# HPC-Research-Lab/GNN

Measured on AMD Instinct MI355X. Metric: mini-batches/sec + SpMM HBM GB/s, Reddit GraphSAGE/LADIES at 1/2/4/8 MI355X, higher is better.
Workload: dtype f32

## Files before the change

### gnn_amd/_lib.py

```python
from __future__ import annotations

import contextlib
import ctypes
import os
import threading

import torch

_HERE = os.path.dirname(os.path.abspath(__file__))
LIB_PATH = os.environ.get("GNN_SPMM_LIBRARY") or os.path.join(_HERE, "libgnn_spmm.so")

_lock = threading.Lock()
_lib = None

c_i32p = ctypes.c_void_p
_VP = ctypes.c_void_p
_I64 = ctypes.c_int64
_SZ = ctypes.c_size_t
_INT = ctypes.c_int

_SIGNATURES = {
    "gnn_last_error": (ctypes.c_char_p, []),
    "gnn_version": (ctypes.c_char_p, []),
    "gnn_spmm_default_unit_nnz": (_I64, [_I64, _I64, _I64]),
    "gnn_spmm_workspace_bytes": (_SZ, [_I64, _I64, _I64, _I64]),
    "gnn_spmm_csr_f32": (_INT, [_VP, _VP, _VP, _I64, _I64, _I64, _VP, _I64, _VP, _I64, _I64, _VP, _SZ, _I64, _VP]),
    "gnn_spmm_csr_f32_ex": (_INT, [_VP, _VP, _VP, _I64, _I64, _I64, _VP, _I64, _VP, _I64, _I64, _VP, _I64, _VP,
                                   _VP, _SZ, _I64, _VP]),
    "gnn_spmm_kernel_name": (_INT, [_I64, _I64, _I64, _I64, _I64, _I64, _VP, _VP, _I64, _INT, ctypes.c_char_p, _SZ]),
    "gnn_spmm_config":(_INT, [_I64, _I64, _I64, _I64, _I64, _I64, _VP, _VP, _I64, ctypes.POINTER(ctypes.c_int32)]),
    "gnn_spmm_csr_h16_f32": (_INT, [_VP, _VP, _VP, _I64, _I64, _I64, _VP, _I64, _INT, _VP, _I64, _I64, _VP, _SZ, _I64,
                                    _VP]),
    "gnn_spmm_h16_config": (_INT, [_I64, _I64, _I64, _I64, _I64, _I64, _VP, _VP, _I64,
                                   ctypes.POINTER(ctypes.c_int32)]),
    "gnn_spmm_graph_workspace_bytes": (_SZ, [_I64, _I64, _I64]),
    "gnn_spmm_graph_f32": (_INT, [_VP, _VP, _VP, _I64, _I64, _I64, _I64, _I64, _VP, _I64, _INT, _VP, _I64, _I64, _VP,
                                  _SZ, _VP]),
    "gnn_spmm_rows_workspace_bytes": (_SZ, [_I64, _I64, _I64]),
    "gnn_spmm_rows_f32": (_INT, [_VP, _VP, _VP, _I64, _VP, _I64, _VP, _I64, _VP, _I64, _VP, _I64, _INT, _VP, _I64, _I64,
                                 _VP, _SZ, _VP, _VP]),
    "gnn_closure_table_bytes": (_SZ, [_I64]),
    "gnn_closure_workspace_bytes": (_SZ, [_I64]),
    "gnn_closure_mark": (_INT, [_VP, _VP, _I64, _VP, _I64, ctypes.c_int32, _VP, _VP, _VP, _SZ, _VP]),
    "gnn_closure_list": (_INT, [_VP, _I64, _VP, _I64, _VP]),
    "gnn_closure_rank": (_INT, [_VP, _I64, _VP, _I64, _VP, _VP, _VP]),
    "gnn_nbr_workspace_bytes": (_SZ, [_I64]),
    "gnn_nbr_rowptr": (_INT, [_VP, _I64, _I64, _VP, _I64, ctypes.c_int32, _VP, _VP, _VP, _SZ, _VP, _VP]),
    "gnn_nbr_draw": (_INT, [_VP, _VP, _I64, _I64, _VP, _I64, ctypes.c_int32, ctypes.c_uint64, ctypes.c_int32, _VP, _VP,
                            _VP, _I64, _VP, _VP]),
    "gnn_nbr_relabel": (_INT, [_VP, _I64, _VP, _I64, _VP, _VP, _VP, _VP]),
    "gnn_lw_race": (_INT, [_VP, _VP, _I64, _I64, _VP, _I64, _VP, ctypes.c_uint64, ctypes.c_int32, _VP, _VP, _I64, _VP,
                           _VP, _VP]),
    "gnn_lw_select_workspace_bytes": (_SZ, []),
    "gnn_lw_select": (_INT, [_VP, _VP, _VP, _I64, _I64, _VP, _VP, _VP, _VP, _VP, _SZ, _VP]),
    "gnn_lw_finish_workspace_bytes": (_SZ, [_I64, _I64]),
    "gnn_lw_finish": (_INT, [_VP, _I64, _VP, _I64, _I64, _VP, _I64, _VP, _VP, _I64, _VP, _VP, _I64, _VP, _VP, _VP, _VP,
                             _VP, _VP, _VP, _VP, _SZ, _VP, _VP]),
    "gnn_spmm_set_timing_events": (None, [_VP, _VP]),
    "gnn_segsort_workspace_bytes": (_SZ, [_I64]),
    "gnn_build_operand_workspace_bytes": (_SZ, []),
    "gnn_build_operand_f32": (_INT, [_VP, _VP, _VP, _INT, _VP, _I64, _I64, _I64, _VP, _VP, _VP, _VP, _SZ, _VP]),
    "gnn_build_operand_t_f32": (_INT, [_VP, _VP, _VP, _VP, _I64, _I64, _I64, _VP, _VP]),
    "gnn_build_operand_sorted_f32": (_INT, [_VP, _VP, _VP, _INT, _VP, _I64, _I64, _I64, _VP, _VP, _VP, _VP]),
    "gnn_coo_to_csr": (_INT, [_VP, _VP, _I64, _I64, _VP, _VP, _VP]),
    "gnn_csr_transpose_workspace_bytes": (_SZ, [_I64, _I64, _I64]),
    "gnn_csr_transpose": (_INT, [_VP, _VP, _VP, _I64, _I64, _I64, _VP, _VP, _VP, _VP, _SZ, _VP]),
    "gnn_gather_rows_f32": (_INT, [_VP, _I64, _VP, _VP, _I64, _VP, _I64, _I64, _VP]),
    "gnn_gather_rows2_f32": (_INT, [_VP, _I64, _VP, _VP, _I64, _VP, _I64, _VP, _VP, _I64, _VP, _I64, _I64, _VP]),
    "gnn_gather_rows_h16_f32": (_INT, [_VP, _I64, _INT, _VP, _VP, _I64, _VP, _I64, _I64, _VP]),
    "gnn_gather_rows2_h16_f32": (_INT, [_VP, _I64, _VP, _VP, _I64, _VP, _I64, _VP, _VP, _I64, _INT, _VP, _I64, _I64,
                                        _VP]),
    "gnn_gather_rows_host_f32": (_INT, [_VP, _I64, _VP, _VP, _I64, _VP, _I64, _I64, _VP]),
    "gnn_gather_placed_f32": (_INT, [_VP, _I64, _VP, _INT, _VP, _I64, _INT, _VP, _I64, _VP, _I64, _I64, _VP, _VP, _VP]),
    "gnn_host_register": (_INT, [_VP, _SZ]),
    "gnn_host_unregister": (_INT, [_VP]),
    "gnn_memcpy_h2d_async": (_INT, [_VP, _VP, _SZ, _VP]),
    "gnn_stage_plan": (_SZ, [_VP, _VP]),
    "gnn_stage_batch_f32": (_INT, [_VP, _VP]),
    "gnn_stream_create_cu_masked": (_INT, [ctypes.c_int32, ctypes.c_int32, ctypes.c_int32, ctypes.POINTER(_VP)]),
    "gnn_stream_destroy": (_INT, [_VP]),
    "gnn_ipc_export": (_INT, [_VP, _VP, ctypes.POINTER(_I64)]),
    "gnn_ipc_open": (_INT, [_VP, _I64, _INT, ctypes.POINTER(_VP)]),
    "gnn_ipc_close": (_INT, [_VP, _I64]),
    "gnn_sage_norm_fwd_f32": (_INT, [_VP, _I64, _I64, _VP, _I64, _I64, _VP, _VP, _VP, _VP, _I64, ctypes.c_float,
                                     ctypes.c_uint64, _INT, _VP, _I64, _VP, _VP, _VP]),
    "gnn_sage_norm_bwd_workspace_bytes": (_SZ, [_I64, _I64]),
    "gnn_sage_norm_bwd_f32": (_INT, [_VP, _I64, _VP, _I64, _I64, _VP, _I64, _I64, _VP, _VP, _VP, _VP, _VP, _I64,
                                     ctypes.c_float, ctypes.c_uint64, _INT, _VP, _VP, _VP, _VP, _VP, _VP, _VP, _SZ,
                                     _VP]),
    "gnn_sage_norm_bwd_agg_f32": (_INT, [_VP, _VP, _VP, _VP, _I64, _VP, _I64, _VP, _VP, _I64, _I64, _VP, _I64, _I64,
                                         _VP, _VP, _VP, _VP, _VP, _I64, ctypes.c_float, ctypes.c_uint64, _INT, _VP,
                                         _VP, _VP, _VP, _VP, _VP, _VP, _SZ, _VP]),
    "gnn_sage_norm_config": (_INT, [_I64, _I64, _INT, ctypes.POINTER(ctypes.c_int), ctypes.POINTER(ctypes.c_int),
                                    ctypes.POINTER(ctypes.c_int)]),
    "gnn_gemm_p3_packed_bytes": (_SZ, [_I64, _I64]),
    "gnn_gemm_p3_pack_f32": (_INT, [_VP, _I64, _INT, _VP, _I64, _I64, _VP, _SZ, _VP]),
    "gnn_gemm_p3_workspace_bytes": (_SZ, [_I64, _I64, _I64, _INT]),
    "gnn_gemm_p3": (_INT, [_I64, _I64, _I64, _INT, _VP, _VP, _VP, _I64, _VP, _SZ, _VP]),
    "gnn_optim_chunks": (_I64, [_INT, _VP]),
    "gnn_grad_sqnorm_f32": (_INT, [_INT, _VP, _VP, _VP, _VP]),
    "gnn_clip_scale_f32": (_INT, [_VP, _I64, ctypes.c_float, _VP, _VP]),
    "gnn_scale_into_f32": (_INT, [_INT, _VP, _VP, _VP, _VP, _VP]),
    "gnn_adam_f32": (_INT, [_INT, _VP, _VP, _VP, _VP, _VP, _VP, ctypes.c_float, ctypes.c_float, ctypes.c_float,
                            ctypes.c_float, _I64, _VP]),
    "gnn_head_bce_fwd_f32": (_INT, [_VP, _I64, _I64, _I64, _VP, _VP, _I64, _VP, _I64, ctypes.c_float,
                                    ctypes.c_uint64, _INT, _VP, _VP, _VP, _VP, _VP, _VP]),
    "gnn_head_bce_bwd_f32": (_INT, [_VP, _I64, _I64, _I64, _VP, _I64, _VP, _I64, _VP, ctypes.c_float,
                                    ctypes.c_uint64, _INT, _VP, _VP, _VP, _VP, _I64, _VP]),
    "gnn_head_bias_grad_f32": (_INT, [_VP, _I64, _I64, _VP, _VP]),
    "gnn_head_eval_f32": (_INT, [_VP, _I64, _I64, _I64, _VP, _VP, _I64, _VP, _I64, _VP, _I64, _VP, _VP, _VP, _VP, _INT,
                                 _VP]),
    "gnn_head_ce_fwd_f32": (_INT, [_VP, _I64, _I64, _I64, _VP, _VP, _I64, _VP, _I64, ctypes.c_float,
                                   ctypes.c_uint64, _INT, _VP, _VP, _VP, _VP, _VP, _VP, _VP]),
    "gnn_head_ce_bwd_f32": (_INT, [_VP, _I64, _I64, _I64, _VP, _I64, _VP, _I64, _VP, ctypes.c_float,
                                   ctypes.c_uint64, _INT, _VP, _VP, _VP, _VP, _I64, _VP, _VP]),
    "gnn_head_eval_loss_f32": (_INT, [_VP, _I64, _I64, _I64, _VP, _VP, _I64, _VP, _I64, _VP, _I64, _VP, _VP, _VP, _VP,
                                      _INT, _INT, _VP]),
    "gnn_ladies_extract_workspace_bytes": (_SZ, [_I64, _I64, _I64, ctypes.c_int32, _I64, _I64]),
    "gnn_colcount_create": (_INT, [ctypes.c_int32, _I64, _VP, _VP, ctypes.POINTER(_VP)]),
    "gnn_colcount_add": (_INT, [_VP, _VP, _I64, ctypes.POINTER(_I64), ctypes.POINTER(_VP), ctypes.POINTER(_VP)]),
    "gnn_colcount_reset": (_INT, [_VP]),
    "gnn_colcount_destroy": (None, [_VP]),
    "gnn_colcount_set_cus": (_INT, [ctypes.c_int32]),
    "gnn_ladies_extract_f32": (_INT, [_VP, _VP, _VP, _I64, _VP, _VP, _VP, _I64, _VP, _I64, _VP, _I64, _VP, _VP, _VP, _I64,
                                      _I64, _VP, _VP, _VP, _VP, _VP, _VP, _SZ, _VP, _VP]),
    "gnn_train_step_workspace_bytes": (_SZ, [_VP]),
    "gnn_train_step_f32": (_INT, [_VP, _VP, _SZ, _VP]),
    "gnn_eval_step_workspace_bytes": (_SZ, [_VP]),
    "gnn_eval_step_f32": (_INT, [_VP, _VP, _I64, _VP, _INT, _VP, _SZ, _VP]),
    "gnn_gemm_f32_workspace_bytes": (_SZ, [_I64, _I64, _I64, _INT]),
    "gnn_gemm_f32": (_INT, [_INT, _INT, _I64, _I64, _I64, _INT, _VP, _I64, _VP, _I64, _VP, _I64, _VP, _SZ, _VP]),
    "gnn_gemm_f32_split3_workspace_bytes": (_SZ, [_I64, _I64, _I64, _INT]),
    "gnn_gemm_f32_split3_indexed": (_INT, [_INT, _INT, _I64, _I64, _I64, _INT, _VP, _I64, _VP, _I64, _VP, _I64, _VP,
                                           _I64, _VP, _I64, _VP, _SZ, _VP]),
    "gnn_gemm_f32_split3": (_INT, [_INT, _INT, _I64, _I64, _I64, _INT, _VP, _I64, _VP, _I64, _VP, _I64, _VP, _SZ,
                                   _VP]),
    "gnn_gemm_f32_split_workspace_bytes": (_SZ, [_INT, _I64, _I64, _I64, _INT]),
    "gnn_gemm_f32_split": (_INT, [_INT, _INT, _INT, _I64, _I64, _I64, _INT, _VP, _I64, _VP, _I64, _VP, _I64, _VP, _SZ,
                                  _VP]),
    "gnn_gemm_f32_split_indexed": (_INT, [_INT, _INT, _INT, _I64, _I64, _I64, _INT, _VP, _I64, _VP, _I64, _VP, _I64,
                                          _VP, _I64, _VP, _I64, _VP, _SZ, _VP]),
}

EXPORTED_SYMBOLS = tuple(_SIGNATURES)

SAMPLER_PATH = os.path.join(_HERE, "libgnn_sampler.so")
_SAMPLER_SIGNATURES = {
    "gnn_sampler_last_error": (ctypes.c_char_p, []),
    "gnn_ladies_sample": (_INT, [_VP, _VP, _VP, _I64, _VP, _I64, _VP, _VP, ctypes.c_int32, ctypes.c_uint32,
                                 ctypes.POINTER(_VP)]),
    "gnn_ladies_sample_dev": (_INT, [_VP, _VP, _VP, _VP, _I64, _VP, _I64, _VP, _VP, ctypes.c_int32, ctypes.c_uint32,
                                     ctypes.c_int32, ctypes.POINTER(_VP)]),
    "gnn_ladies_layer_device": (_INT, [_VP, ctypes.c_int32, _VP, _VP, _VP, _VP, _VP]),
    "gnn_subgraph_sample": (_INT, [_VP, _VP, _VP, _I64, _VP, _I64, _VP, _VP, ctypes.c_int32, ctypes.c_uint32,
                                   ctypes.POINTER(_VP)]),
    "gnn_fastgcn_sample": (_INT, [_VP, _VP, _VP, _I64, _VP, _VP, _I64, _VP, _VP, ctypes.c_int32, ctypes.c_uint32,
                                  ctypes.POINTER(_VP)]),
    "gnn_fastgcn_p_changed": (None, []),
    "gnn_ladies_layer_dims": (_INT, [_VP, ctypes.c_int32, ctypes.POINTER(_I64)]),
    "gnn_ladies_layer_copy": (_INT, [_VP, ctypes.c_int32, _VP, _VP, _VP, _VP, _VP]),
    "gnn_ladies_layer_csc": (_INT, [_VP, ctypes.c_int32, _VP, _VP]),
    "gnn_ladies_num_input_nodes": (_I64, [_VP]),
    "gnn_ladies_input_nodes": (_INT, [_VP, _VP]),
    "gnn_ladies_free": (None, [_VP]),
    "gnn_mt19937_random_sample": (_INT, [ctypes.c_uint32, _I64, _VP]),
    "gnn_sampler_profile": (_INT, [_VP, ctypes.c_int32, ctypes.c_int32]),
    "gnn_host_gather_rows_f32": (_INT, [_VP, _I64, _I64, _VP, _I64, _I64, _VP, _I64]),
    "gnn_host_gather_rows_b16": (_INT, [_VP, _I64, _I64, _VP, _I64, _I64, _VP, _I64]),
    "gnn_loader_set_feat_b16": (_INT, [_VP, _VP, _I64, _I64, _I64, ctypes.c_int32]),
    "gnn_loader_create": (_VP, [_VP, _VP, _VP, _VP, _I64, _VP, _VP, _VP, _I64, _VP, _VP, ctypes.c_int32, ctypes.c_int32,
                                _VP, _VP, _I64, _I64, _I64, _VP, _VP, ctypes.c_int32, ctypes.c_int32, _VP,
                                ctypes.c_int32, ctypes.c_int32, ctypes.c_int32, ctypes.c_int32]),
    "gnn_loader_submit": (_INT, [_VP, ctypes.c_uint32, _VP, _I64]),
    "gnn_loader_set_colcount": (_INT, [_VP, _VP]),
    "gnn_loader_set_colcount_workers": (_INT, [_VP, ctypes.c_int32]),
    "gnn_ladies_sample_cc": (_INT, [_VP, _VP, _VP, _VP, _I64, _VP, _I64, _VP, _VP, ctypes.c_int32, ctypes.c_uint32,
                                    ctypes.c_int32, _VP, _VP, ctypes.POINTER(_VP)]),
    "gnn_loader_next": (_INT, [_VP, ctypes.POINTER(_VP)]),
    "gnn_batch_desc": (ctypes.POINTER(_I64), [_VP, ctypes.POINTER(_I64)]),
    "gnn_batch_blob": (_VP, [_VP]),
    "gnn_batch_release": (None, [_VP]),
    "gnn_loader_destroy": (None, [_VP]),
}
SAMPLER_EXPORTED_SYMBOLS = tuple(_SAMPLER_SIGNATURES)
_sampler = None


def lib() -> ctypes.CDLL:
    global _lib
    if _lib is not None:
        return _lib
    with _lock:
        if _lib is None:
            if not os.path.exists(LIB_PATH):
                raise RuntimeError(
                    f"gnn_amd: native library {LIB_PATH} is missing; build it with "
                    "`python -c 'import __graft_entry__ as g; g.build()'` (hipcc, gfx950)")
            handle = ctypes.CDLL(LIB_PATH)
            for name, (res, args) in _SIGNATURES.items():
                fn = getattr(handle, name)
                fn.restype = res
                fn.argtypes = args
            _lib = handle
    return _lib


def sampler_lib() -> ctypes.CDLL:
    global _sampler
    if _sampler is not None:
        return _sampler
    with _lock:
        if _sampler is None:
            if not os.path.exists(SAMPLER_PATH):
                raise RuntimeError(f"gnn_amd: native sampler {SAMPLER_PATH} is missing; build it with "
                                   "`python -c 'import __graft_entry__ as g; g.build()'`")
            handle = ctypes.CDLL(SAMPLER_PATH)
            for name, (res, args) in _SAMPLER_SIGNATURES.items():
                fn = getattr(handle, name)
                fn.restype = res
                fn.argtypes = args
            _sampler = handle
    return _sampler


def check_sampler(rc: int, what: str) -> None:
    if rc != 0:
        msg = sampler_lib().gnn_sampler_last_error().decode(errors="replace")
        raise RuntimeError(f"{what} failed (status {rc}): {msg}")


_NULLCTX = contextlib.nullcontext()


def stream_of(dev) -> int:
    return torch._C._cuda_getCurrentRawStream(dev.index if dev.index is not None else torch.cuda.current_device())


def on_device(dev):
    if dev.index is None or dev.index == torch._C._cuda_getDevice():
        return _NULLCTX
    return torch.cuda.device(dev)


def check(rc: int, what: str) -> None:
    if rc != 0:
        msg = lib().gnn_last_error().decode(errors="replace")
        raise RuntimeError(f"{what} failed (status {rc}): {msg}")
```

### gnn_amd/csrc/common.h

```cpp
#pragma once

#include <hip/hip_runtime.h>

#include <cstddef>
#include <cstdint>

#define GNN_EINVAL (-22)

namespace gnn {

int fail(int code, const char* fmt, ...);

inline size_t align_up(size_t x, size_t a) { return (x + a - 1) / a * a; }
inline int64_t ceil_div(int64_t a, int64_t b) { return (a + b - 1) / b; }

inline int pick_vw(int64_t F, int64_t ldx, int64_t ldy, const void* X, const void* Y) {
  const uintptr_t px = (uintptr_t)X, py = (uintptr_t)Y;
  if (F % 4 == 0 && ldx % 4 == 0 && ldy % 4 == 0 && px % 16 == 0 && py % 16 == 0) return 4;
  if (F % 2 == 0 && ldx % 2 == 0 && ldy % 2 == 0 && px % 8 == 0 && py % 8 == 0) return 2;
  return 1;
}

int launch_scan_exclusive(const int* in, int n, int* out, hipStream_t st);

bool spmm_row_chain(int64_t M, int64_t K, int64_t nnz, int64_t F, int64_t ldx, int64_t ldy, const void* X,
                    const void* Y);

int gemm_split3_as_batch(int a_kmajor, int b_kmajor, int64_t M, int64_t N, int64_t K, int nbatch, int split_nbatch,
                         int batch_index, const float* const* A, int64_t lda, const float* const* B, int64_t ldb,
                         float* const* C, int64_t ldc, void* workspace, size_t workspace_bytes, void* stream,
                         int pieces = 3);

int gemm_split3_indexed(int a_kmajor, int b_kmajor, int64_t M, int64_t N, int64_t K, int nbatch,
                        const float* const* A, int64_t lda, const int64_t* const* ia, int64_t a_rows,
                        const float* const* B, int64_t ldb, const int64_t* const* ib, int64_t b_rows,
                        float* const* C, int64_t ldc, void* workspace, size_t workspace_bytes, void* stream,
                        int pieces = 3);

}

#define GNN_REQUIRE(cond, ...)                              \
  do {                                                      \
    if (!(cond)) return ::gnn::fail(GNN_EINVAL, __VA_ARGS__); \
  } while (0)

#define GNN_LAUNCHED(name)                                                                       \
  do {                                                                                           \
    hipError_t e_ = hipGetLastError();                                                           \
    if (e_ != hipSuccess) return ::gnn::fail((int)e_, "%s launch: %s", name, hipGetErrorString(e_)); \
  } while (0)

#define GNN_HIP(call, name)                                                                \
  do {                                                                                     \
    hipError_t e_ = (call);                                                                \
    if (e_ != hipSuccess) {                                                                \
      (void)hipGetLastError();                                                             \
      return ::gnn::fail((int)e_, "%s: %s", name, hipGetErrorString(e_));                  \
    }                                                                                      \
  } while (0)
```

### gnn_amd/csrc/gemm.hip

```cpp
#include <hip/hip_runtime.h>

#include <algorithm>
#include <climits>
#include <cstdint>
#include <cstdlib>

#include "common.h"
#include "gnn_layers.h"

namespace {

using gnn::ceil_div;

typedef float f2 __attribute__((ext_vector_type(2)));
typedef float f4 __attribute__((ext_vector_type(4)));
typedef float f16v __attribute__((ext_vector_type(16)));

constexpr int BM = 128, BN = 128;
constexpr int KM_LD = BM + 32;
constexpr int MAX_BATCH = 4;

template <int BKT>
struct Stage {
  static constexpr int MM_LD = BKT + 2;
  static constexpr int FLOATS = (BKT * KM_LD > BM * MM_LD) ? BKT * KM_LD : BM * MM_LD;
  static constexpr int NP = BKT / 8;
};

struct Batch {
  const float* A[MAX_BATCH];
  const float* B[MAX_BATCH];
  float* C[MAX_BATCH];
  const int64_t* ia[MAX_BATCH];
  const int64_t* ib[MAX_BATCH];
};

template <int VEC>
__device__ __forceinline__ f4 load4(const float* p) {
  if constexpr (VEC == 4) {
    return *reinterpret_cast<const f4*>(p);
  } else {
    const f2 lo = *reinterpret_cast<const f2*>(p);
    const f2 hi = *reinterpret_cast<const f2*>(p + 2);
    return f4{lo.x, lo.y, hi.x, hi.y};
  }
}

template <bool KMAJ, int VEC, int BKT, bool GUARD>
__device__ __forceinline__ void load_tile(const float* __restrict__ P, int64_t ld, int r0, int rlim, int k0, int klim,
                                          int t, f4 v[Stage<BKT>::NP]) {
#pragma unroll
  for (int j = 0; j < Stage<BKT>::NP; ++j) {
    if constexpr (KMAJ) {
      const int k = k0 + (t >> 5) + 8 * j;
      const int m = r0 + (t & 31) * 4;
      if constexpr (!GUARD) {
        const float* row = P + (int64_t)k * ld;
        if constexpr (VEC == 4) {
          v[j] = load4<4>(row + min(m, ((rlim - 1) >> 2) << 2));
        } else {
          const int mc = ((rlim - 1) >> 1) << 1;
          const f2 lo = *reinterpret_cast<const f2*>(row + min(m, mc));
          const f2 hi = *reinterpret_cast<const f2*>(row + min(m + 2, mc));
          v[j] = f4{lo.x, lo.y, hi.x, hi.y};
        }
      } else {
        f4 x = f4(0.0f);
        if (k < klim) {
          const float* row = P + (int64_t)k * ld;
          if (m + 0 < rlim) x.x = row[m + 0];
          if (m + 1 < rlim) x.y = row[m + 1];
          if (m + 2 < rlim) x.z = row[m + 2];
          if (m + 3 < rlim) x.w = row[m + 3];
        }
        v[j] = x;
      }
    } else {
      constexpr int TPR = BKT / 4;
      const int m = min(r0 + t / TPR + (256 / TPR) * j, rlim - 1);
      const int k = k0 + (t % TPR) * 4;
      const float* q = P + (int64_t)m * ld + k;
      if constexpr (!GUARD) {
        v[j] = load4<VEC>(q);
      } else {
        f4 x = f4(0.0f);
        if (k + 0 < klim) x.x = q[0];
        if (k + 1 < klim) x.y = q[1];
        if (k + 2 < klim) x.z = q[2];
        if (k + 3 < klim) x.w = q[3];
        v[j] = x;
      }
    }
  }
}

template <bool KMAJ, int BKT>
__device__ __forceinline__ void store_tile(float* __restrict__ S, int t, const f4 v[Stage<BKT>::NP]) {
#pragma unroll
  for (int j = 0; j < Stage<BKT>::NP; ++j) {
    if constexpr (KMAJ) {
      const int kk = (t >> 5) + 8 * j, m = (t & 31) * 4;
      *reinterpret_cast<f4*>(S + kk * KM_LD + m) = v[j];
    } else {
      constexpr int TPR = BKT / 4;
      const int m = t / TPR + (256 / TPR) * j, kk = (t % TPR) * 4;
      float* p = S + m * Stage<BKT>::MM_LD + kk;
      *reinterpret_cast<f2*>(p) = f2{v[j].x, v[j].y};
      *reinterpret_cast<f2*>(p + 2) = f2{v[j].z, v[j].w};
    }
  }
}

template <bool KMAJ, int BKT>
__device__ __forceinline__ float frag(const float* __restrict__ S, int r, int k) {
  if constexpr (KMAJ) return S[k * KM_LD + r];
  else return S[r * Stage<BKT>::MM_LD + k];
}

template <int NB>
__device__ __forceinline__ void store_acc(const f16v (&acc)[2][NB], float* Cb, int64_t ldo, int M, int N, int m0,
                                          int n0, int wm, int wn, int li, int lh) {
#pragma unroll
  for (int i = 0; i < 2; ++i) {
#pragma unroll
    for (int j = 0; j < NB; ++j) {
      const int n = n0 + wn * (32 * NB) + j * 32 + li;
      if (n >= N) continue;
#pragma unroll
      for (int r = 0; r < 16; ++r) {
        const int m = (m0 + wm * 64 + i * 32 + (r & 3) + 8 * (r >> 2)) | (4 * lh);
        if (m < M) Cb[(int64_t)m * ldo + n] = acc[i][j][r];
      }
    }
  }
}

template <bool AK, bool BKM, int VA, int VB, int BKT>
__global__ __launch_bounds__(256) void gemm_f32_kernel(Batch bt, int M, int N, int K, int64_t lda, int64_t ldb,
                                                          int64_t ldc, int splits, int klen, float* __restrict__ part) {
  __shared__ __attribute__((aligned(16))) float As[2][Stage<BKT>::FLOATS];
  __shared__ __attribute__((aligned(16))) float Bs[2][Stage<BKT>::FLOATS];
  const int t = threadIdx.x;
  const int lane = t & 63;
  const int wid = t >> 6;
  const int wm = wid >> 1, wn = wid & 1;
  const int b = blockIdx.z / splits;
  const int split = blockIdx.z % splits;
  const int m0 = blockIdx.y * BM;
  const int n0 = blockIdx.x * BN;
  const int kbeg = split * klen;
  const int kend = min(K, kbeg + klen);
  const float* __restrict__ A = bt.A[b];
  const float* __restrict__ B = bt.B[b];

  f16v acc[2][2];
#pragma unroll
  for (int i = 0; i < 2; ++i)
#pragma unroll
    for (int j = 0; j < 2; ++j) acc[i][j] = f16v(0.0f);

  const int nk = kend > kbeg ? (kend - kbeg + BKT - 1) / BKT : 0;
  f4 ra[Stage<BKT>::NP], rb[Stage<BKT>::NP];
  auto load_ab = [&](int k0) {
    if (k0 + BKT <= kend) {
      load_tile<AK, VA, BKT, false>(A, lda, m0, M, k0, kend, t, ra);
      load_tile<BKM, VB, BKT, false>(B, ldb, n0, N, k0, kend, t, rb);
    } else {
      load_tile<AK, VA, BKT, true>(A, lda, m0, M, k0, kend, t, ra);
      load_tile<BKM, VB, BKT, true>(B, ldb, n0, N, k0, kend, t, rb);
    }
  };
  if (nk > 0) {
    load_ab(kbeg);
    store_tile<AK, BKT>(As[0], t, ra);
    store_tile<BKM, BKT>(Bs[0], t, rb);
  }
  __syncthreads();
  const int li = lane & 31, lk = lane >> 5;
  for (int kt = 0; kt < nk; ++kt) {
    const int cur = kt & 1;
    if (kt + 1 < nk) load_ab(kbeg + (kt + 1) * BKT);
    const float* Sa = As[cur];
    const float* Sb = Bs[cur];
#pragma unroll
    for (int s = 0; s < BKT / 2; ++s) {
      const int k = 2 * s + lk;
      const float a0 = frag<AK, BKT>(Sa, wm * 64 + li, k);
      const float a1 = frag<AK, BKT>(Sa, wm * 64 + 32 + li, k);
      const float b0 = frag<BKM, BKT>(Sb, wn * 64 + li, k);
      const float b1 = frag<BKM, BKT>(Sb, wn * 64 + 32 + li, k);
      acc[0][0] = __builtin_amdgcn_mfma_f32_32x32x2f32(a0, b0, acc[0][0], 0, 0, 0);
      acc[0][1] = __builtin_amdgcn_mfma_f32_32x32x2f32(a0, b1, acc[0][1], 0, 0, 0);
      acc[1][0] = __builtin_amdgcn_mfma_f32_32x32x2f32(a1, b0, acc[1][0], 0, 0, 0);
      acc[1][1] = __builtin_amdgcn_mfma_f32_32x32x2f32(a1, b1, acc[1][1], 0, 0, 0);
    }
    if (kt + 1 < nk) {
      store_tile<AK, BKT>(As[cur ^ 1], t, ra);
      store_tile<BKM, BKT>(Bs[cur ^ 1], t, rb);
    }
    __syncthreads();
  }
  store_acc<2>(acc, splits > 1 ? part + (int64_t)blockIdx.z * M * N : bt.C[b], splits > 1 ? N : ldc, M, N, m0, n0, wm,
               wn, li, lk);
}

__global__ __launch_bounds__(256) void gemm_splitk_reduce4_kernel(Batch bt, const float* __restrict__ part, int64_t MN,
                                                                  int splits, int nbatch) {
  const int64_t n4 = MN / 4;
  for (int64_t e = (int64_t)blockIdx.x * 256 + threadIdx.x; e < n4 * nbatch; e += (int64_t)gridDim.x * 256) {
    const int b = (int)(e / n4);
    const int64_t o = (e - (int64_t)b * n4) * 4;
    const float* p = part + (int64_t)b * splits * MN + o;
    f4 acc = *reinterpret_cast<const f4*>(p);
    int q = 1;
    for (; q + 3 < splits; q += 4) {
      const f4 v0 = *reinterpret_cast<const f4*>(p + (int64_t)q * MN);
      const f4 v1 = *reinterpret_cast<const f4*>(p + (int64_t)(q + 1) * MN);
      const f4 v2 = *reinterpret_cast<const f4*>(p + (int64_t)(q + 2) * MN);
      const f4 v3 = *reinterpret_cast<const f4*>(p + (int64_t)(q + 3) * MN);
      acc += v0;
      acc += v1;
      acc += v2;
      acc += v3;
    }
    for (; q < splits; ++q) acc += *reinterpret_cast<const f4*>(p + (int64_t)q * MN);
    *reinterpret_cast<f4*>(bt.C[b] + o) = acc;
  }
}

__global__ __launch_bounds__(256) void gemm_splitk_reduce_kernel(Batch bt, const float* __restrict__ part, int M, int N,
                                                                 int64_t ldc, int splits, int nbatch) {
  const int64_t MN = (int64_t)M * N;
  for (int64_t e = (int64_t)blockIdx.x * 256 + threadIdx.x; e < MN * nbatch; e += (int64_t)gridDim.x * 256) {
    const int b = (int)(e / MN);
    const int64_t o = e - (int64_t)b * MN;
    const float* p = part + (int64_t)b * splits * MN + o;
    float s = p[0];
    for (int q = 1; q < splits; ++q) s += p[(int64_t)q * MN];
    const int m = (int)(o / N), n = (int)(o - (int64_t)m * N);
    bt.C[b][(int64_t)m * ldc + n] = s;
  }
}

typedef __bf16 bf8v __attribute__((ext_vector_type(8)));
typedef unsigned int u4v __attribute__((ext_vector_type(4)));

constexpr int S3_BK = 16;
constexpr int S3_PIECE = BM * S3_BK;
constexpr int S3_OPER = 3 * S3_PIECE;

__device__ __forceinline__ __amdgpu_buffer_rsrc_t s3_rsrc(const float* p, int64_t bytes) {
  return __builtin_amdgcn_make_buffer_rsrc((void*)p, (short)0, (int)bytes, 0x00020000);
}

template <bool KMAJ, int VEC, bool GUARD, bool IX = false>
__device__ __forceinline__ void s3_load(__amdgpu_buffer_rsrc_t rs, const float* __restrict__ P, int64_t ld, int voff,
                                        int r0, int rlim, int k0, int klim, int t, float v[8],
                                        const int64_t* __restrict__ idx = nullptr) {
  if constexpr (KMAJ) {
    const int kb = k0 + __builtin_amdgcn_readfirstlane((t >> 7) * 8);
    if constexpr (GUARD) {
      const int m = min(r0 + (t & 127), rlim - 1);
#pragma unroll
      for (int i = 0; i < 8; ++i)
        v[i] = (kb + i < klim) ? P[(IX ? idx[kb + i] : (int64_t)(kb + i)) * ld + m] : 0.0f;
    } else {
#pragma unroll
      for (int i = 0; i < 8; ++i)
        v[i] = __builtin_bit_cast(
            float, __builtin_amdgcn_raw_buffer_load_b32(
                       rs, voff, (int)((IX ? idx[kb + i] : (int64_t)(kb + i)) * ld * 4), 0));
    }
  } else {
    if constexpr (GUARD) {
      const int m = min(r0 + (t >> 1), rlim - 1);
      const int kb = k0 + (t & 1) * 8;
      const float* q = P + (IX ? idx[m] : (int64_t)m) * ld + kb;
#pragma unroll
      for (int i = 0; i < 8; ++i) v[i] = (kb + i < klim) ? q[i] : 0.0f;
    } else {
      const int so = k0 * 4;
      if constexpr (VEC == 4) {
        const f4 a = __builtin_bit_cast(f4, __builtin_amdgcn_raw_buffer_load_b128(rs, voff, so, 0));
        const f4 b = __builtin_bit_cast(f4, __builtin_amdgcn_raw_buffer_load_b128(rs, voff + 16, so, 0));
        v[0] = a.x; v[1] = a.y; v[2] = a.z; v[3] = a.w;
        v[4] = b.x; v[5] = b.y; v[6] = b.z; v[7] = b.w;
      } else {
#pragma unroll
        for (int i = 0; i < 4; ++i) {
          const f2 a = __builtin_bit_cast(f2, __builtin_amdgcn_raw_buffer_load_b64(rs, voff + 8 * i, so, 0));
          v[2 * i] = a.x;
          v[2 * i + 1] = a.y;
        }
      }
    }
  }
}

template <bool KMAJ>
__device__ __forceinline__ int s3_voff(int64_t ld, int r0, int rlim, int t, const int64_t* __restrict__ idx = nullptr) {
  if constexpr (KMAJ) return min(r0 + (t & 127), rlim - 1) * 4;
  else {
    const int r = min(r0 + (t >> 1), rlim - 1);
    return (int)(((idx ? idx[r] : (int64_t)r) * ld + (t & 1) * 8) * 4);
  }
}

template <bool KMAJ, int R>
__device__ __forceinline__ int s3_chunk(int row, int h) {
  if constexpr (KMAJ) return (h * R + row) * 8;
  else return (2 * row + (h ^ ((row >> 3) & 1))) * 8;
}

typedef __bf16 bf2v __attribute__((ext_vector_type(2)));

__device__ __forceinline__ unsigned int rne_pk(float a, float b) {
  return __builtin_bit_cast(unsigned int, __builtin_convertvector(f2{a, b}, bf2v));
}

template <int NP = 3>
__device__ __forceinline__ void split8(const float v[8], u4v& ph, u4v& pm, u4v& pl) {
  if constexpr (NP == 1) {
#pragma unroll
    for (int j = 0; j < 4; ++j) ph[j] = rne_pk(v[2 * j], v[2 * j + 1]);
    return;
  } else if constexpr (NP == 2) {
#pragma unroll
    for (int j = 0; j < 4; ++j) {
      const float x0 = v[2 * j], x1 = v[2 * j + 1];
      const unsigned int h0 = (__float_as_uint(x0) + 0x80u) & 0xffff0000u;
      const unsigned int h1 = (__float_as_uint(x1) + 0x80u) & 0xffff0000u;
      const float r0 = __builtin_amdgcn_fmed3f(x0 - __uint_as_float(h0), 0.0f, x0);
      const float r1 = __builtin_amdgcn_fmed3f(x1 - __uint_as_float(h1), 0.0f, x1);
      ph[j] = __builtin_amdgcn_perm(h1, h0, 0x07060302u);
      pm[j] = rne_pk(r0, r1);
    }
    return;
  }
#pragma unroll
  for (int j = 0; j < 4; ++j) {
    const float x0 = v[2 * j], x1 = v[2 * j + 1];
    const unsigned int h0 = __float_as_uint(x0) & 0xffff0000u, h1 = __float_as_uint(x1) & 0xffff0000u;
    const float r0 = x0 - __uint_as_float(h0), r1 = x1 - __uint_as_float(h1);
    const unsigned int m0 = __float_as_uint(r0) & 0xffff0000u, m1 = __float_as_uint(r1) & 0xffff0000u;
    const float l0 = r0 - __uint_as_float(m0), l1 = r1 - __uint_as_float(m1);
    ph[j] = __builtin_amdgcn_perm(h1, h0, 0x07060302u);
    pm[j] = __builtin_amdgcn_perm(m1, m0, 0x07060302u);
    pl[j] = __builtin_amdgcn_perm(__float_as_uint(l1), __float_as_uint(l0), 0x07060302u);
  }
}

template <bool KMAJ, int R, int NP = 3>
__device__ __forceinline__ void s3_store(unsigned short* __restrict__ S, int rr, int kh, const float v[8]) {
  u4v ph, pm, pl;
  split8<NP>(v, ph, pm, pl);
  const int off = s3_chunk<KMAJ, R>(rr, kh);
  *reinterpret_cast<u4v*>(S + off) = ph;
  if constexpr (NP >= 2) *reinterpret_cast<u4v*>(S + R * S3_BK + off) = pm;
  if constexpr (NP >= 3) *reinterpret_cast<u4v*>(S + 2 * R * S3_BK + off) = pl;
}

template <bool KMAJ, int R, int NP = 3>
__device__ __forceinline__ void s3_store(unsigned short* __restrict__ S, int t, const float v[8]) {
  s3_store<KMAJ, R, NP>(S, KMAJ ? (t & 127) : (t >> 1), KMAJ ? (t >> 7) : (t & 1), v);
}

template <bool KMAJ, int R>
__device__ __forceinline__ bf8v s3_frag(const unsigned short* __restrict__ S, int piece, int row, int h) {
  return __builtin_bit_cast(bf8v, *reinterpret_cast<const u4v*>(S + piece * R * S3_BK + s3_chunk<KMAJ, R>(row, h)));
}

constexpr int s3_products(int np) { return np == 3 ? 6 : np == 2 ? 4 : 1; }
constexpr int s3_piece_a(int np, int q) {
  constexpr int P3[6] = {2, 1, 0, 1, 0, 0}, P2[4] = {1, 1, 0, 0};
  return np == 3 ? P3[q] : np == 2 ? P2[q] : 0;
}
constexpr int s3_piece_b(int np, int q) {
  constexpr int P3[6] = {0, 1, 2, 0, 1, 0}, P2[4] = {1, 0, 1, 0};
  return np == 3 ? P3[q] : np == 2 ? P2[q] : 0;
}

template <bool AK, bool BKM, int NB, int NP = 3>
__device__ __forceinline__ void s3_mma(const unsigned short* __restrict__ Sa, const unsigned short* __restrict__ Sb,
                                       int ra0, int rb0, int li, int lh, f16v (&acc)[2][NB]) {
  constexpr int G = NB == 2 ? 2 : 1;
  bf8v a[2][NP], bb[G][NP];
#pragma unroll
  for (int p = 0; p < NP; ++p)
#pragma unroll
    for (int i = 0; i < 2; ++i) {
      a[i][p] = s3_frag<AK, BM>(Sa, p, ra0 + i * 32 + li, lh);
      if constexpr (G == 2) bb[i][p] = s3_frag<BKM, 64 * NB>(Sb, p, rb0 + i * 32 + li, lh);
    }
#pragma unroll
  for (int j0 = 0; j0 < NB; j0 += G) {
    if constexpr (G == 1) {
#pragma unroll
      for (int p = 0; p < NP; ++p) bb[0][p] = s3_frag<BKM, 64 * NB>(Sb, p, rb0 + j0 * 32 + li, lh);
    }
#pragma unroll
    for (int q = 0; q < s3_products(NP); ++q)
#pragma unroll
      for (int i = 0; i < 2; ++i)
#pragma unroll
        for (int g = 0; g < G; ++g)
          acc[i][j0 + g] = __builtin_amdgcn_mfma_f32_32x32x16_bf16(a[i][s3_piece_a(NP, q)], bb[g][s3_piece_b(NP, q)],
                                                                  acc[i][j0 + g], 0, 0, 0);
  }
}

__device__ __forceinline__ int3 xcd_tile(int gx, int gy, unsigned gz, unsigned bx, unsigned by, unsigned bz) {
  const int total = gx * gy * gz;
  const int hw = bx + gx * (by + gy * bz);
  const int per = total >> 3;
  const int lg = hw < per * 8 ? (hw & 7) * per + (hw >> 3) : hw;
  return make_int3(lg % gx, (lg / gx) % gy, lg / (gx * gy));
}

template <bool AK, bool BKM, int VA, int VB, bool IDX, int NB, int NP = 3>
__global__ __launch_bounds__(256)
    __attribute__((amdgpu_waves_per_eu(NB == 2 ? 3 : 2, NB == 2 ? (NP == 3 ? 3 : 4) : 2))) void
gemm_s3_kernel(Batch bt, int M, int N, int K, int64_t lda, int64_t ldb, int64_t ldc, int splits, int klen,
               float* __restrict__ part, int64_t abytes, int64_t bbytes, int xcd_map, int tail_base = 0,
               int tail_s = 0) {
  constexpr int TN = 64 * NB;
  constexpr int NH = NB / 2;
  static_assert(NP >= 1 && NP <= 3 && (NP == 3 || NB == 2), "reduced piece counts: the 128 x 128 tile only");
  __shared__ __attribute__((aligned(16))) unsigned short As[2][NP * S3_PIECE];
  __shared__ __attribute__((aligned(16))) unsigned short Bs[2][NH * NP * S3_PIECE];
  const int t = threadIdx.x;
  const int lane = t & 63;
  const int wid = t >> 6;
  const int wm = wid >> 1, wn = wid & 1;
  int tx = blockIdx.x, ty = blockIdx.y, tz = blockIdx.z;
  int b, split;
  int piece = -1;
  if (NB == 2 && tail_s > 0) {
    const int gx = (N + BN - 1) / BN, gy = (M + BM - 1) / BM;
    const int hw = blockIdx.x;
    int lg;
    if (hw < tail_base) {
      const int per = tail_base >> 3;
      lg = xcd_map ? (hw & 7) * per + (hw >> 3) : hw;
      split = 0;
    } else {
      piece = hw - tail_base;
      lg = tail_base + piece / tail_s;
      split = piece % tail_s;
    }
    tx = lg % gx;
    ty = (lg / gx) % gy;
    b = lg / (gx * gy);
  } else {
    if (xcd_map) {
      const int3 tile = xcd_tile(gridDim.x, gridDim.y, gridDim.z, blockIdx.x, blockIdx.y, blockIdx.z);
      tx = tile.x, ty = tile.y, tz = tile.z;
    }
    b = tz / splits;
    split = tz % splits;
  }
  const int m0 = ty * BM;
  const int n0 = tx * TN;
  const bool whole = NB == 2 && tail_s > 0 && piece < 0;
  const int kbeg = whole ? 0 : split * klen;
  const int kend = whole ? K : min(K, kbeg + klen);
  const float* __restrict__ A = bt.A[b];
  const float* __restrict__ B = bt.B[b];
  const __amdgpu_buffer_rsrc_t rsa = s3_rsrc(A, abytes), rsb = s3_rsrc(B, bbytes);
  const int64_t* __restrict__ ia = (IDX && !AK) ? bt.ia[b] : nullptr;
  const int64_t* __restrict__ ib = (IDX && BKM) ? bt.ib[b] : nullptr;
  const int voa = s3_voff<AK>(lda, m0, M, t, ia);
  const int vob0 = s3_voff<BKM>(ldb, n0, N, t);
  const int vob1 = NH == 2 ? s3_voff<BKM>(ldb, n0 + BN, N, t) : 0;

  const int ar = AK ? (t & 127) : (t >> 1), ah = AK ? (t >> 7) : (t & 1);
  const int br = BKM ? (t & 127) : (t >> 1), bh = BKM ? (t >> 7) : (t & 1);
  f16v acc[2][NB];
#pragma unroll
  for (int i = 0; i < 2; ++i)
#pragma unroll
    for (int j = 0; j < NB; ++j) acc[i][j] = f16v(0.0f);

  float ra[2][8], rb[2][8 * NH];
  const int nfull = (kend - kbeg) / S3_BK;
  auto load_ab = [&](int kt, float(&xa)[8], float(&xb)[8 * NH]) {
    const int k0 = kbeg + min(kt, nfull - 1) * S3_BK;
    s3_load<AK, VA, false>(rsa, A, lda, voa, m0, M, k0, kend, t, xa);
    if (IDX && BKM && ib)
      s3_load<BKM, VB, false, true>(rsb, B, ldb, vob0, n0, N, k0, kend, t, xb, ib);
    else
      s3_load<BKM, VB, false>(rsb, B, ldb, vob0, n0, N, k0, kend, t, xb);
    if constexpr (NH == 2) {
      if (IDX && BKM && ib)
        s3_load<BKM, VB, false, true>(rsb, B, ldb, vob1, n0 + BN, N, k0, kend, t, xb + 8, ib);
      else
        s3_load<BKM, VB, false>(rsb, B, ldb, vob1, n0 + BN, N, k0, kend, t, xb + 8);
    }
  };
  auto store_ab = [&](int stage, const float(&xa)[8], const float(&xb)[8 * NH]) {
    if constexpr (NH == 2) {
      s3_store<AK, BM, NP>(As[stage], ar, ah, xa);
      s3_store<BKM, TN, NP>(Bs[stage], br, bh, xb);
      s3_store<BKM, TN, NP>(Bs[stage], br + BN, bh, xb + 8);
    } else {
      s3_store<AK, BM, NP>(As[stage], t, xa);
      s3_store<BKM, TN, NP>(Bs[stage], t, xb);
    }
  };
  const int li = lane & 31, lh = lane >> 5;
  if (nfull > 0) {
    load_ab(0, ra[0], rb[0]);
    load_ab(1, ra[1], rb[1]);
    store_ab(0, ra[0], rb[0]);
    __syncthreads();
    int kt = 0;
    for (; kt + 1 < nfull; kt += 2) {
      load_ab(kt + 2, ra[0], rb[0]);
      s3_mma<AK, BKM, NB, NP>(As[0], Bs[0], wm * 64, wn * (32 * NB), li, lh, acc);
      store_ab(1, ra[1], rb[1]);
      __syncthreads();
      load_ab(kt + 3, ra[1], rb[1]);
      s3_mma<AK, BKM, NB, NP>(As[1], Bs[1], wm * 64, wn * (32 * NB), li, lh, acc);
      store_ab(0, ra[0], rb[0]);
      __syncthreads();
    }
    if (nfull & 1) {
      s3_mma<AK, BKM, NB, NP>(As[0], Bs[0], wm * 64, wn * (32 * NB), li, lh, acc);
      __syncthreads();
    }
  }
  if (kbeg + nfull * S3_BK < kend) {
    const int k0 = kbeg + nfull * S3_BK;
    if (IDX && !AK && ia)
      s3_load<AK, VA, true, true>(rsa, A, lda, voa, m0, M, k0, kend, t, ra[0], ia);
    else
      s3_load<AK, VA, true>(rsa, A, lda, voa, m0, M, k0, kend, t, ra[0]);
    if (IDX && BKM && ib)
      s3_load<BKM, VB, true, true>(rsb, B, ldb, vob0, n0, N, k0, kend, t, rb[0], ib);
    else
      s3_load<BKM, VB, true>(rsb, B, ldb, vob0, n0, N, k0, kend, t, rb[0]);
    if constexpr (NH == 2) {
      if (IDX && BKM && ib)
        s3_load<BKM, VB, true, true>(rsb, B, ldb, vob1, n0 + BN, N, k0, kend, t, rb[0] + 8, ib);
      else
        s3_load<BKM, VB, true>(rsb, B, ldb, vob1, n0 + BN, N, k0, kend, t, rb[0] + 8);
    }
    store_ab(0, ra[0], rb[0]);
    __syncthreads();
    s3_mma<AK, BKM, NB, NP>(As[0], Bs[0], wm * 64, wn * (32 * NB), li, lh, acc);
  }

  if constexpr (NB == 2) {
    if (piece >= 0) {
      float* __restrict__ P = part + (int64_t)piece * (BM * BN);
#pragma unroll
      for (int i = 0; i < 2; ++i)
#pragma unroll
        for (int j = 0; j < 2; ++j)
#pragma unroll
          for (int r = 0; r < 16; ++r)
            P[(wm * 64 + i * 32 + (r & 3) + 8 * (r >> 2) + 4 * lh) * BN + wn * 64 + j * 32 + li] = acc[i][j][r];
      return;
    }
  }
  store_acc<NB>(acc, splits > 1 ? part + (int64_t)tz * M * N : bt.C[b], splits > 1 ? N : ldc, M, N, m0, n0, wm, wn, li,
                lh);
}


__global__ __launch_bounds__(256) void gemm_tail_reduce_kernel(Batch bt, const float* __restrict__ part, int M, int N,
                                                               int64_t ldc, int tail_base, int tail_s) {
  const int tile = blockIdx.x >> 4;
  const int e4 = (blockIdx.x & 15) * 256 + threadIdx.x;
  const int ml = e4 >> 5, nl = (e4 & 31) * 4;
  const float* p = part + (int64_t)tile * tail_s * (BM * BN) + ml * BN + nl;
  f4 acc = *reinterpret_cast<const f4*>(p);
  for (int q = 1; q < tail_s; ++q) acc += *reinterpret_cast<const f4*>(p + (int64_t)q * (BM * BN));
  const int gx = (N + BN - 1) / BN, gy = (M + BM - 1) / BM;
  const int lg = tail_base + tile;
  const int m = ((lg / gx) % gy) * BM + ml, n = (lg % gx) * BN + nl;
  if (m >= M) return;
  float* c = bt.C[lg / (gx * gy)] + (int64_t)m * ldc + n;
  if (n + 0 < N) c[0] = acc.x;
  if (n + 1 < N) c[1] = acc.y;
  if (n + 2 < N) c[2] = acc.z;
  if (n + 3 < N) c[3] = acc.w;
}

__global__ __launch_bounds__(256) void p3_pack_kernel(const float* __restrict__ src, int64_t ld, int kmajor,
                                                      const int64_t* __restrict__ idx, int R, int K, int Rp, int KT,
                                                      unsigned short* __restrict__ out) {
  const int t = threadIdx.x;
  const int r0 = blockIdx.x * 128;
  const int kt = blockIdx.y;
  const int rr = kmajor ? (t & 127) : (t >> 1);
  const int kh = kmajor ? (t >> 7) : (t & 1);
  const int r = r0 + rr;
  const int kb = kt * 16 + kh * 8;
  float v[8];
  if (!kmajor) {
    const float* q = (r < R) ? src + (idx ? idx[r] : (int64_t)r) * ld : nullptr;
#pragma unroll
    for (int i = 0; i < 8; ++i) v[i] = (q && kb + i < K) ? q[kb + i] : 0.0f;
  } else {
#pragma unroll
    for (int i = 0; i < 8; ++i) {
      const int k = kb + i;
      v[i] = (r < R && k < K) ? src[(idx ? idx[k] : (int64_t)k) * ld + r] : 0.0f;
    }
  }
  u4v ph, pm, pl;
  split8(v, ph, pm, pl);
  const int64_t plane = (int64_t)KT * Rp * 16;
  const int64_t o = ((int64_t)kt * Rp + r) * 16 + kh * 8;
  *reinterpret_cast<u4v*>(out + o) = ph;
  *reinterpret_cast<u4v*>(out + plane + o) = pm;
  *reinterpret_cast<u4v*>(out + 2 * plane + o) = pl;
}

struct PBatch {
  const unsigned short* A[MAX_BATCH];
  const unsigned short* B[MAX_BATCH];
  float* C[MAX_BATCH];
};

__global__ __launch_bounds__(256) __attribute__((amdgpu_waves_per_eu(3, 3))) void gemm_p3_kernel(
    PBatch bt, int M, int N, int Mp, int Np, int KT, int64_t ldc, int splits, int ktlen, float* __restrict__ part,
    int xcd_map) {
  __shared__ __attribute__((aligned(16))) unsigned short As[2][S3_OPER];
  __shared__ __attribute__((aligned(16))) unsigned short Bs[2][S3_OPER];
  const int t = threadIdx.x;
  const int lane = t & 63;
  const int wid = t >> 6;
  const int wm = wid >> 1, wn = wid & 1;
  int tx = blockIdx.x, ty = blockIdx.y, tz = blockIdx.z;
  if (xcd_map) {
    const int3 tile = xcd_tile(gridDim.x, gridDim.y, gridDim.z, blockIdx.x, blockIdx.y, blockIdx.z);
    tx = tile.x, ty = tile.y, tz = tile.z;
  }
  const int b = tz / splits;
  const int split = tz % splits;
  const int m0 = ty * BM;
  const int n0 = tx * BN;
  const int ktb = split * ktlen;
  const int kte = min(KT, ktb + ktlen);
  const int64_t aplane = (int64_t)KT * Mp * 16, bplane = (int64_t)KT * Np * 16;
  const __amdgpu_buffer_rsrc_t rsa = __builtin_amdgcn_make_buffer_rsrc((void*)bt.A[b], (short)0,
                                                                      (int)(3 * aplane * 2), 0x00020000);
  const __amdgpu_buffer_rsrc_t rsb = __builtin_amdgcn_make_buffer_rsrc((void*)bt.B[b], (short)0,
                                                                      (int)(3 * bplane * 2), 0x00020000);
  const int rr = t >> 1, kh = t & 1;
  const int voa = ((m0 + rr) * 16 + kh * 8) * 2, vob = ((n0 + rr) * 16 + kh * 8) * 2;
  const int off = s3_chunk<false, BM>(rr, kh);

  f16v acc[2][2];
#pragma unroll
  for (int i = 0; i < 2; ++i)
#pragma unroll
    for (int j = 0; j < 2; ++j) acc[i][j] = f16v(0.0f);

  u4v ra[2][3], rb[2][3];
  const int nfull = kte - ktb;
  auto load_ab = [&](int kt, u4v(&xa)[3], u4v(&xb)[3]) {
    const int k = ktb + min(kt, nfull - 1);
#pragma unroll
    for (int p = 0; p < 3; ++p) {
      xa[p] = __builtin_bit_cast(u4v, __builtin_amdgcn_raw_buffer_load_b128(
                                          rsa, voa, (int)((p * aplane + (int64_t)k * Mp * 16) * 2), 0));
      xb[p] = __builtin_bit_cast(u4v, __builtin_amdgcn_raw_buffer_load_b128(
                                          rsb, vob, (int)((p * bplane + (int64_t)k * Np * 16) * 2), 0));
    }
  };
  auto store_ab = [&](int stage, const u4v(&xa)[3], const u4v(&xb)[3]) {
#pragma unroll
    for (int p = 0; p < 3; ++p) {
      *reinterpret_cast<u4v*>(As[stage] + p * S3_PIECE + off) = xa[p];
      *reinterpret_cast<u4v*>(Bs[stage] + p * S3_PIECE + off) = xb[p];
    }
  };
  const int li = lane & 31, lh = lane >> 5;
  if (nfull > 0) {
    load_ab(0, ra[0], rb[0]);
    load_ab(1, ra[1], rb[1]);
    store_ab(0, ra[0], rb[0]);
    __syncthreads();
    int kt = 0;
    for (; kt + 1 < nfull; kt += 2) {
      load_ab(kt + 2, ra[0], rb[0]);
      s3_mma<false, false, 2>(As[0], Bs[0], wm * 64, wn * 64, li, lh, acc);
      store_ab(1, ra[1], rb[1]);
      __syncthreads();
      load_ab(kt + 3, ra[1], rb[1]);
      s3_mma<false, false, 2>(As[1], Bs[1], wm * 64, wn * 64, li, lh, acc);
      store_ab(0, ra[0], rb[0]);
      __syncthreads();
    }
    if (nfull & 1) {
      s3_mma<false, false, 2>(As[0], Bs[0], wm * 64, wn * 64, li, lh, acc);
      __syncthreads();
    }
  }
  store_acc<2>(acc, splits > 1 ? part + (int64_t)tz * M * N : bt.C[b], splits > 1 ? N : ldc, M, N, m0, n0, wm, wn, li, lh);
}

constexpr int64_t SLOTS_F32 = 2 * 256;
constexpr int64_t SLOTS_S3 = 3 * 256;

int pick_splits(int64_t M, int64_t N, int64_t K, int nbatch, int64_t tile_n, int64_t slots) {
  if (const char* e = getenv("GNN_GEMM_SPLITS")) return std::max(1, atoi(e));
  const int64_t tiles = ceil_div(M, (int64_t)BM) * ceil_div(N, tile_n) * nbatch;
  if (tiles * 2 > slots) return 1;
  int64_t s = slots / tiles;
  s = std::min<int64_t>(s, std::max<int64_t>(1, K / 256));
  return (int)std::max<int64_t>(1, std::min<int64_t>(s, 64));
}

constexpr int W_BN = 2 * BN;
constexpr int64_t SLOTS_S3W = 2 * 256;

bool use_wide(int64_t M, int64_t N, int64_t K, int nbatch) {
  const char* e = getenv("GNN_GEMM_WIDE");
  const int mode = e ? atoi(e) : 0;
  if (mode == 0 || N < W_BN || K <= 0) return false;
  if (mode == 1) return true;
  if (getenv("GNN_GEMM_SPLITS")) return false;
  const int64_t tw = ceil_div(M, (int64_t)BM) * ceil_div(N, (int64_t)W_BN) * nbatch;
  return tw * 100 >= SLOTS_S3W * 85 && tw <= SLOTS_S3W;
}

struct TailPlan {
  int base = 0;
  int s = 0;
  int rem = 0;
};

TailPlan tail_plan(int64_t M, int64_t N, int64_t K, int nbatch) {
  TailPlan tp;
  const int64_t T = ceil_div(M, (int64_t)BM) * ceil_div(N, (int64_t)BN) * nbatch;
  if (T <= 256 || T >= INT_MAX / 2) return tp;
  const int64_t rem = T % 256;
  if (rem == 0 || rem > 32) return tp;
  const int64_t S = std::min<int64_t>(std::min<int64_t>(256 / rem, 4), ceil_div(K, (int64_t)16) / 4);
  if (S < 2) return tp;
  tp.base = (int)(T - rem);
  tp.s = (int)S;
  tp.rem = (int)rem;
  return tp;
}

bool tail_enabled() {
  const char* e = getenv("GNN_GEMM_TAIL");
  return !(e && atoi(e) == 0);
}

size_t tail_bytes(const TailPlan& tp) { return (size_t)tp.rem * tp.s * BM * BN * sizeof(float); }

enum Algo { ALGO_F32 = 0, ALGO_S3 = 1 };
enum Kern { KERN_F32, KERN_S3, KERN_S3W };

bool xcd_map_enabled() {
  const char* e = getenv("GNN_GEMM_XCD");
  return !e || atoi(e) != 0;
}

struct Plan {
  Kern kern = KERN_F32;
  int splits = 1;
  TailPlan tp;
  size_t bytes(int64_t M, int64_t N, int nbatch) const {
    return splits > 1 ? (size_t)splits * nbatch * M * N * sizeof(float) : tail_bytes(tp);
  }
};

Plan plan_of(int algo, int64_t M, int64_t N, int64_t K, int nbatch, int split_nbatch = 0, int batch_index = -1,
             int pieces = 3) {
  const int nb = split_nbatch > 0 ? split_nbatch : nbatch;
  Plan p;
  p.kern = algo != ALGO_S3 ? KERN_F32 : (pieces == 3 && use_wide(M, N, K, nb)) ? KERN_S3W : KERN_S3;
  if (K > 0)
    p.splits = p.kern == KERN_S3W   ? pick_splits(M, N, K, nb, W_BN, SLOTS_S3W)
               : p.kern == KERN_S3 ? pick_splits(M, N, K, nb, BN, SLOTS_S3)
                                   : pick_splits(M, N, K, nb, BN, SLOTS_F32);
  if (p.kern != KERN_S3 || p.splits > 1 || K <= 0) return p;
  if (split_nbatch == 0) {
    p.tp = tail_plan(M, N, K, nbatch);
  } else if (nbatch == 1 && batch_index >= 0) {
    const TailPlan full = tail_plan(M, N, K, split_nbatch);
    const int64_t T1 = ceil_div(M, (int64_t)BM) * ceil_div(N, (int64_t)BN);
    const int64_t lo = (int64_t)batch_index * T1;
    if (full.s > 0 && full.base < lo + T1) {
      p.tp.base = (int)std::max<int64_t>(0, full.base - lo);
      p.tp.s = full.s;
      p.tp.rem = (int)(T1 - p.tp.base);
    }
  }
  return p;
}

size_t workspace_bytes_of(int algo, int64_t M, int64_t N, int64_t K, int nbatch, int pieces = 3) {
  if (M <= 0 || N <= 0 || K <= 0 || nbatch <= 0) return 0;
  return plan_of(algo, M, N, K, nbatch, 0, -1, pieces).bytes(M, N, nbatch);
}

int launch_splitk_reduce(const Batch& bt, const float* part, int64_t M, int64_t N, int64_t ldc, int splits, int nbatch,
                         hipStream_t st) {
  const int64_t total = M * N * nbatch;
  bool vec4 = ldc == N && (M * N) % 4 == 0;
  for (int b = 0; b < nbatch; ++b) vec4 = vec4 && (uintptr_t)bt.C[b] % 16 == 0;
  if (vec4) {
    const unsigned g = (unsigned)std::min<int64_t>(ceil_div(total / 4, (int64_t)256), 2048);
    gemm_splitk_reduce4_kernel<<<dim3(g), dim3(256), 0, st>>>(bt, part, M * N, splits, nbatch);
    GNN_LAUNCHED("gemm_splitk_reduce4_kernel");
  } else {
    const unsigned g = (unsigned)std::min<int64_t>(ceil_div(total, (int64_t)256), 2048);
    gemm_splitk_reduce_kernel<<<dim3(g), dim3(256), 0, st>>>(bt, part, (int)M, (int)N, ldc, splits, nbatch);
    GNN_LAUNCHED("gemm_splitk_reduce_kernel");
  }
  return 0;
}

struct Launch {
  Kern kern;
  bool idx;
  int np;
  int bkt;
  dim3 grid;
  hipStream_t st;
  Batch bt;
  int M, N, K;
  int64_t lda, ldb, ldc;
  int splits, klen;
  float* part;
  int64_t abytes, bbytes;
  int xcdm, tail_base, tail_s;
};

template <bool AK, bool BKM, int VA, int VB, int NP>
void launch_s3_reduced(const Launch& l) {
  auto k = gemm_s3_kernel<AK, BKM, VA, VB, false, 2, NP>;
  if constexpr (!AK || BKM)
    if (l.idx) k = gemm_s3_kernel<AK, BKM, VA, VB, true, 2, NP>;
  k<<<l.grid, dim3(256), 0, l.st>>>(l.bt, l.M, l.N, l.K, l.lda, l.ldb, l.ldc, l.splits, l.klen, l.part, l.abytes,
                                    l.bbytes, l.xcdm, l.tail_base, l.tail_s);
}

template <bool AK, bool BKM, int VA, int VB>
void launch_gemm(const Launch& l) {
  if (l.kern == KERN_F32) {
    auto k = l.bkt == 16 ? gemm_f32_kernel<AK, BKM, VA, VB, 16> : gemm_f32_kernel<AK, BKM, VA, VB, 32>;
    k<<<l.grid, dim3(256), 0, l.st>>>(l.bt, l.M, l.N, l.K, l.lda, l.ldb, l.ldc, l.splits, l.klen, l.part);
    return;
  }
  if (l.np < 3) {
    constexpr int CVA = AK ? 4 : VA, CVB = BKM ? 4 : VB;
    if (l.np == 2) launch_s3_reduced<AK, BKM, CVA, CVB, 2>(l);
    else launch_s3_reduced<AK, BKM, CVA, CVB, 1>(l);
    return;
  }
  const bool wide = l.kern == KERN_S3W;
  auto k = wide ? gemm_s3_kernel<AK, BKM, VA, VB, false, 4> : gemm_s3_kernel<AK, BKM, VA, VB, false, 2>;
  if constexpr (!AK || BKM)
    if (l.idx) k = wide ? gemm_s3_kernel<AK, BKM, VA, VB, true, 4> : gemm_s3_kernel<AK, BKM, VA, VB, true, 2>;
  k<<<l.grid, dim3(256), 0, l.st>>>(l.bt, l.M, l.N, l.K, l.lda, l.ldb, l.ldc, l.splits, l.klen, l.part, l.abytes,
                                    l.bbytes, l.xcdm, l.tail_base, l.tail_s);
}

template <bool AK, bool BKM>
void launch_gemm(int va, int vb, const Launch& l) {
  if (va == 4 && vb == 4) launch_gemm<AK, BKM, 4, 4>(l);
  else if (va == 4) launch_gemm<AK, BKM, 4, 2>(l);
  else if (vb == 4) launch_gemm<AK, BKM, 2, 4>(l);
  else launch_gemm<AK, BKM, 2, 2>(l);
}

struct RowIndex {
  const int64_t* const* ia = nullptr;
  int64_t a_rows = 0;
  const int64_t* const* ib = nullptr;
  int64_t b_rows = 0;
};

int gemm_run(int algo, int a_kmajor, int b_kmajor, int64_t M, int64_t N, int64_t K, int nbatch, const float* const* A,
             int64_t lda, const float* const* B, int64_t ldb, float* const* C, int64_t ldc, void* workspace,
             size_t workspace_bytes, void* stream, int split_nbatch = 0, const RowIndex* ri = nullptr,
             int batch_index = -1, int pieces = 3) {
  GNN_REQUIRE(pieces >= 1 && pieces <= 3 && (pieces == 3 || algo == ALGO_S3),
              "gnn_gemm_f32_split: pieces %d (1: bf16, 2: split2, 3: split3)", pieces);
  GNN_REQUIRE(M >= 0 && N >= 0 && K >= 0, "gnn_gemm_f32: negative size");
  GNN_REQUIRE(M < INT_MAX && N < INT_MAX && K < INT_MAX, "gnn_gemm_f32: sizes must be < 2^31");
  GNN_REQUIRE(nbatch >= 1 && nbatch <= MAX_BATCH, "gnn_gemm_f32: nbatch must be 1..%d", MAX_BATCH);
  if (M == 0 || N == 0) return 0;
  GNN_REQUIRE(A && B && C, "gnn_gemm_f32: NULL pointer array");
  GNN_REQUIRE(ldc >= N, "gnn_gemm_f32: ldc < N");
  GNN_REQUIRE(lda >= (a_kmajor ? M : K) && ldb >= (b_kmajor ? N : K), "gnn_gemm_f32: lda/ldb too small");
  GNN_REQUIRE(lda % 2 == 0 && ldb % 2 == 0, "gnn_gemm_f32: lda and ldb must be even (8-byte rows)");
  Launch l{};
  Batch& bt = l.bt;
  int va = 4, vb = 4;
  for (int b = 0; b < nbatch; ++b) {
    GNN_REQUIRE(C[b] && (K == 0 || (A[b] && B[b])), "gnn_gemm_f32: NULL operand %d", b);
    GNN_REQUIRE((uintptr_t)A[b] % 8 == 0 && (uintptr_t)B[b] % 8 == 0, "gnn_gemm_f32: A/B not 8-byte aligned");
    if (lda % 4 || (uintptr_t)A[b] % 16) va = 2;
    if (ldb % 4 || (uintptr_t)B[b] % 16) vb = 2;
    bt.A[b] = A[b];
    bt.B[b] = B[b];
    bt.C[b] = C[b];
    bt.ia[b] = ri && ri->ia ? ri->ia[b] : nullptr;
    bt.ib[b] = ri && ri->ib ? ri->ib[b] : nullptr;
  }
  for (int b = 0; b < nbatch; ++b) l.idx = l.idx || bt.ia[b] || bt.ib[b];
  GNN_REQUIRE(!l.idx || (algo == ALGO_S3 && (!ri->ia || !a_kmajor) && (!ri->ib || b_kmajor)),
              "gnn_gemm: row indices need split3, an m-major A or a k-major B");
  const int64_t arows = (ri && ri->ia) ? ri->a_rows : (a_kmajor ? K : M);
  const int64_t brows = (ri && ri->ib) ? ri->b_rows : (b_kmajor ? K : N);
  l.abytes = K == 0 ? 0 : (arows - 1) * lda * 4 + (a_kmajor ? M : K) * 4;
  l.bbytes = K == 0 ? 0 : (brows - 1) * ldb * 4 + (b_kmajor ? N : K) * 4;
  if (algo == ALGO_S3 && (l.abytes >= INT_MAX || l.bbytes >= INT_MAX)) {
    GNN_REQUIRE(!l.idx, "gnn_gemm: indexed operand of >= 2 GiB");
    GNN_REQUIRE(pieces == 3, "gnn_gemm_f32_split: operand of >= 2 GiB at %d pieces", pieces);
    algo = ALGO_F32;
  }
  l.np = pieces;
  Plan pl = plan_of(algo, M, N, K, nbatch, split_nbatch, batch_index, pieces);
  if (!tail_enabled()) pl.tp = TailPlan{};
  const TailPlan& tp = pl.tp;
  l.kern = pl.kern;
  l.splits = pl.splits;
  l.xcdm = xcd_map_enabled() && !(tp.s > 0 && tp.base % 8);
  l.bkt = algo == ALGO_S3 ? S3_BK : 32;
  if (algo == ALGO_F32)
    if (const char* e = getenv("GNN_GEMM_BKT")) l.bkt = atoi(e) == 16 ? 16 : 32;
  const int64_t kpart = tp.s > 0 ? tp.s : l.splits;
  l.klen = kpart > 1 ? (int)(ceil_div(ceil_div(K, kpart), (int64_t)l.bkt) * l.bkt) : (int)K;
  if (l.splits > 1 || tp.s > 0) {
    const size_t need = pl.bytes(M, N, nbatch);
    GNN_REQUIRE(workspace && workspace_bytes >= need, "gnn_gemm_f32: workspace too small (%zu < %zu)",
                workspace_bytes, need);
  }
  l.grid = tp.s > 0 ? dim3((unsigned)(tp.base + tp.rem * tp.s))
                    : dim3((unsigned)ceil_div(N, (int64_t)(l.kern == KERN_S3W ? W_BN : BN)),
                           (unsigned)ceil_div(M, (int64_t)BM), (unsigned)(nbatch * l.splits));
  l.st = (hipStream_t)stream;
  l.M = (int)M, l.N = (int)N, l.K = (int)K;
  l.lda = lda, l.ldb = ldb, l.ldc = ldc;
  l.part = (float*)workspace;
  l.tail_base = tp.base, l.tail_s = tp.s;
  if (a_kmajor && b_kmajor) launch_gemm<true, true>(va, vb, l);
  else if (a_kmajor) launch_gemm<true, false>(va, vb, l);
  else if (b_kmajor) launch_gemm<false, true>(va, vb, l);
  else launch_gemm<false, false>(va, vb, l);
  GNN_LAUNCHED(algo == ALGO_S3 ? "gemm_s3_kernel" : "gemm_f32_kernel");
  if (tp.s > 0) {
    gemm_tail_reduce_kernel<<<dim3((unsigned)(tp.rem * 16)), dim3(256), 0, l.st>>>(bt, l.part, (int)M, (int)N, ldc,
                                                                                  tp.base, tp.s);
    GNN_LAUNCHED("gemm_tail_reduce_kernel");
  }
  if (l.splits > 1) return launch_splitk_reduce(bt, l.part, M, N, ldc, l.splits, nbatch, l.st);
  return 0;
}

}

extern "C" {

size_t gnn_gemm_f32_workspace_bytes(int64_t M, int64_t N, int64_t K, int nbatch) {
  return workspace_bytes_of(ALGO_F32, M, N, K, nbatch);
}

int gnn_gemm_f32(int a_kmajor, int b_kmajor, int64_t M, int64_t N, int64_t K, int nbatch, const float* const* A,
                 int64_t lda, const float* const* B, int64_t ldb, float* const* C, int64_t ldc, void* workspace,
                 size_t workspace_bytes, void* stream) {
  return gemm_run(ALGO_F32, a_kmajor, b_kmajor, M, N, K, nbatch, A, lda, B, ldb, C, ldc, workspace, workspace_bytes,
                  stream);
}

size_t gnn_gemm_p3_packed_bytes(int64_t R, int64_t K) {
  if (R <= 0 || K <= 0) return 0;
  return (size_t)3 * (size_t)ceil_div(K, (int64_t)16) * (size_t)(ceil_div(R, (int64_t)128) * 128) * 16 * 2;
}

int gnn_gemm_p3_pack_f32(const float* src, int64_t ld, int kmajor, const int64_t* idx, int64_t R, int64_t K,
                         void* out, size_t out_bytes, void* stream) {
  GNN_REQUIRE(R >= 0 && K >= 0 && R < INT_MAX && K < INT_MAX, "gnn_gemm_p3_pack_f32: bad size");
  if (R == 0 || K == 0) return 0;
  GNN_REQUIRE(src && out, "gnn_gemm_p3_pack_f32: NULL pointer");
  GNN_REQUIRE(out_bytes >= gnn_gemm_p3_packed_bytes(R, K), "gnn_gemm_p3_pack_f32: output too small");
  GNN_REQUIRE((uintptr_t)out % 16 == 0, "gnn_gemm_p3_pack_f32: output not 16-byte aligned");
  GNN_REQUIRE(gnn_gemm_p3_packed_bytes(R, K) < (size_t)INT_MAX, "gnn_gemm_p3_pack_f32: packed operand >= 2 GiB");
  const int Rp = (int)(ceil_div(R, (int64_t)128) * 128), KT = (int)ceil_div(K, (int64_t)16);
  p3_pack_kernel<<<dim3((unsigned)(Rp / 128), (unsigned)KT), dim3(256), 0, (hipStream_t)stream>>>(
      src, ld, kmajor, idx, (int)R, (int)K, Rp, KT, (unsigned short*)out);
  GNN_LAUNCHED("p3_pack_kernel");
  return 0;
}

size_t gnn_gemm_p3_workspace_bytes(int64_t M, int64_t N, int64_t K, int nbatch) {
  return workspace_bytes_of(ALGO_S3, M, N, K, nbatch);
}

int gnn_gemm_p3(int64_t M, int64_t N, int64_t K, int nbatch, const void* const* Ap, const void* const* Bp,
                float* const* C, int64_t ldc, void* workspace, size_t workspace_bytes, void* stream) {
  GNN_REQUIRE(M >= 0 && N >= 0 && K >= 0 && M < INT_MAX && N < INT_MAX && K < INT_MAX, "gnn_gemm_p3: bad size");
  GNN_REQUIRE(nbatch >= 1 && nbatch <= MAX_BATCH, "gnn_gemm_p3: nbatch must be 1..%d", MAX_BATCH);
  if (M == 0 || N == 0) return 0;
  GNN_REQUIRE(Ap && Bp && C && ldc >= N, "gnn_gemm_p3: NULL pointer array or ldc < N");
  PBatch bt{};
  for (int b = 0; b < nbatch; ++b) {
    GNN_REQUIRE(C[b] && (K == 0 || (Ap[b] && Bp[b])), "gnn_gemm_p3: NULL operand %d", b);
    GNN_REQUIRE((uintptr_t)Ap[b] % 16 == 0 && (uintptr_t)Bp[b] % 16 == 0, "gnn_gemm_p3: packed operands 16-byte aligned");
    bt.A[b] = (const unsigned short*)Ap[b];
    bt.B[b] = (const unsigned short*)Bp[b];
    bt.C[b] = C[b];
  }
  GNN_REQUIRE(gnn_gemm_p3_packed_bytes(M, K) < (size_t)INT_MAX && gnn_gemm_p3_packed_bytes(N, K) < (size_t)INT_MAX,
              "gnn_gemm_p3: packed operand >= 2 GiB");
  hipStream_t st = (hipStream_t)stream;
  const int Mp = (int)(ceil_div(M, (int64_t)128) * 128), Np = (int)(ceil_div(N, (int64_t)128) * 128);
  const int KT = (int)ceil_div(K, (int64_t)16);
  const int splits = K == 0 ? 1 : pick_splits(M, N, K, nbatch, BN, SLOTS_S3);
  const int ktlen = splits > 1 ? (int)ceil_div(ceil_div(K, (int64_t)splits), (int64_t)S3_BK) : KT;
  if (splits > 1) {
    const size_t need = (size_t)splits * nbatch * M * N * sizeof(float);
    GNN_REQUIRE(workspace && workspace_bytes >= need, "gnn_gemm_p3: workspace too small (%zu < %zu)", workspace_bytes,
                need);
  }
  const dim3 grid((unsigned)(Np / BN), (unsigned)(Mp / BM), (unsigned)(nbatch * splits));
  float* part = (float*)workspace;
  gemm_p3_kernel<<<grid, dim3(256), 0, st>>>(bt, (int)M, (int)N, Mp, Np, KT, ldc, splits, ktlen, part,
                                             (int)xcd_map_enabled());
  GNN_LAUNCHED("gemm_p3_kernel");
  if (splits > 1) {
    Batch cb{};
    for (int b = 0; b < nbatch; ++b) cb.C[b] = C[b];
    return launch_splitk_reduce(cb, part, M, N, ldc, splits, nbatch, st);
  }
  return 0;
}

size_t gnn_gemm_f32_split3_workspace_bytes(int64_t M, int64_t N, int64_t K, int nbatch) {
  return workspace_bytes_of(ALGO_S3, M, N, K, nbatch);
}

int gnn_gemm_f32_split3(int a_kmajor, int b_kmajor, int64_t M, int64_t N, int64_t K, int nbatch,
                        const float* const* A, int64_t lda, const float* const* B, int64_t ldb, float* const* C,
                        int64_t ldc, void* workspace, size_t workspace_bytes, void* stream) {
  return gemm_run(ALGO_S3, a_kmajor, b_kmajor, M, N, K, nbatch, A, lda, B, ldb, C, ldc, workspace, workspace_bytes,
                  stream);
}

int gnn_gemm_f32_split3_indexed(int a_kmajor, int b_kmajor, int64_t M, int64_t N, int64_t K, int nbatch,
                                const float* const* A, int64_t lda, const int64_t* const* ia, int64_t a_rows,
                                const float* const* B, int64_t ldb, const int64_t* const* ib, int64_t b_rows,
                                float* const* C, int64_t ldc, void* workspace, size_t workspace_bytes, void* stream) {
  GNN_REQUIRE((!ia || a_rows > 0) && (!ib || b_rows > 0), "gnn_gemm_f32_split3_indexed: source rows");
  return gnn::gemm_split3_indexed(a_kmajor, b_kmajor, M, N, K, nbatch, A, lda, ia, a_rows, B, ldb, ib, b_rows, C, ldc,
                                  workspace, workspace_bytes, stream);
}

size_t gnn_gemm_f32_split_workspace_bytes(int pieces, int64_t M, int64_t N, int64_t K, int nbatch) {
  if (pieces < 1 || pieces > 3) return 0;
  return workspace_bytes_of(ALGO_S3, M, N, K, nbatch, pieces);
}

int gnn_gemm_f32_split(int pieces, int a_kmajor, int b_kmajor, int64_t M, int64_t N, int64_t K, int nbatch,
                       const float* const* A, int64_t lda, const float* const* B, int64_t ldb, float* const* C,
                       int64_t ldc, void* workspace, size_t workspace_bytes, void* stream) {
  return gemm_run(ALGO_S3, a_kmajor, b_kmajor, M, N, K, nbatch, A, lda, B, ldb, C, ldc, workspace, workspace_bytes,
                  stream, 0, nullptr, -1, pieces);
}

int gnn_gemm_f32_split_indexed(int pieces, int a_kmajor, int b_kmajor, int64_t M, int64_t N, int64_t K, int nbatch,
                               const float* const* A, int64_t lda, const int64_t* const* ia, int64_t a_rows,
                               const float* const* B, int64_t ldb, const int64_t* const* ib, int64_t b_rows,
                               float* const* C, int64_t ldc, void* workspace, size_t workspace_bytes, void* stream) {
  GNN_REQUIRE(pieces >= 1 && pieces <= 3, "gnn_gemm_f32_split_indexed: pieces %d (1: bf16, 2: split2, 3: split3)",
              pieces);
  GNN_REQUIRE((!ia || a_rows > 0) && (!ib || b_rows > 0), "gnn_gemm_f32_split_indexed: source rows");
  return gnn::gemm_split3_indexed(a_kmajor, b_kmajor, M, N, K, nbatch, A, lda, ia, a_rows, B, ldb, ib, b_rows, C, ldc,
                                  workspace, workspace_bytes, stream, pieces);
}

}

namespace gnn {

int gemm_split3_as_batch(int a_kmajor, int b_kmajor, int64_t M, int64_t N, int64_t K, int nbatch, int split_nbatch,
                         int batch_index, const float* const* A, int64_t lda, const float* const* B, int64_t ldb,
                         float* const* C, int64_t ldc, void* workspace, size_t workspace_bytes, void* stream,
                         int pieces) {
  return gemm_run(ALGO_S3, a_kmajor, b_kmajor, M, N, K, nbatch, A, lda, B, ldb, C, ldc, workspace, workspace_bytes,
                  stream, split_nbatch, nullptr, batch_index, pieces);
}

int gemm_split3_indexed(int a_kmajor, int b_kmajor, int64_t M, int64_t N, int64_t K, int nbatch,
                        const float* const* A, int64_t lda, const int64_t* const* ia, int64_t a_rows,
                        const float* const* B, int64_t ldb, const int64_t* const* ib, int64_t b_rows,
                        float* const* C, int64_t ldc, void* workspace, size_t workspace_bytes, void* stream,
                        int pieces) {
  RowIndex ri;
  ri.ia = ia;
  ri.a_rows = a_rows;
  ri.ib = ib;
  ri.b_rows = b_rows;
  return gemm_run(ALGO_S3, a_kmajor, b_kmajor, M, N, K, nbatch, A, lda, B, ldb, C, ldc, workspace, workspace_bytes,
                  stream, 0, &ri, -1, pieces);
}

}
```

### gnn_amd/csrc/step.hip

```cpp
#include <hip/hip_runtime.h>
#include <rocblas/rocblas.h>

#include <algorithm>
#include <climits>
#include <cstdint>
#include <cstdlib>
#include <cstring>
#include <memory>
#include <mutex>
#include <string>

#include "common.h"
#include "gnn_layers.h"
#include "gnn_spmm.h"
#include "gnn_step.h"

namespace {

using gnn::align_up;
using gnn::ceil_div;

__global__ __launch_bounds__(256) void colsum_kernel(const float* __restrict__ dz, int M, int C,
                                                     float* __restrict__ out) {
  __shared__ float red[4];
  const int c = blockIdx.x;
  float s = 0.0f;
  for (int r = threadIdx.x; r < M; r += 256) s += dz[(int64_t)r * C + c];
#pragma unroll
  for (int m = 32; m >= 1; m >>= 1) s += __shfl_xor(s, m);
  if ((threadIdx.x & 63) == 0) red[threadIdx.x >> 6] = s;
  __syncthreads();
  if (threadIdx.x == 0) out[c] = (red[0] + red[1]) + (red[2] + red[3]);
}

struct Arena {
  char* base;
  size_t off = 0;
  template <typename T>
  T* take(int64_t count) {
    const size_t bytes = align_up((size_t)(count > 0 ? count : 1) * sizeof(T), 256);
    T* p = base ? (T*)(base + off) : nullptr;
    off += bytes;
    return p;
  }
};

int64_t L(const int64_t* d, int l, int f) { return d[GNN_STEP_HEADER + l * GNN_STEP_LAYER_SLOTS + f]; }
template <typename T>
T* P(const int64_t* d, int l, int f) {
  return (T*)(uintptr_t)L(d, l, f);
}
template <typename T>
T* HP(const int64_t* d, int f) {
  return (T*)(uintptr_t)d[f];
}

bool fills(int64_t M, int64_t N, int n) { return ceil_div(M, 128) * ceil_div(N, 128) * n >= 256; }
bool gemm_ok(const void* p, int64_t ld) { return ((uintptr_t)p % 8) == 0 && (ld % 2) == 0; }

std::mutex g_blas_mu;
rocblas_handle g_blas[64][2] = {};

int blas_handle(rocblas_handle* h, int which = 0) {
  int dev = 0;
  GNN_HIP(hipGetDevice(&dev), "hipGetDevice");
  GNN_REQUIRE(dev >= 0 && dev < 64, "gnn_train_step: device index %d", dev);
  std::lock_guard<std::mutex> g(g_blas_mu);
  if (!g_blas[dev][which]) {
    if (rocblas_create_handle(&g_blas[dev][which]) != rocblas_status_success)
      return gnn::fail(-1, "rocblas_create_handle failed");
  }
  *h = g_blas[dev][which];
  return 0;
}

struct Aux {
  hipStream_t s = nullptr;
  hipEvent_t ev[24] = {};
  int next = 0;
  std::mutex mu;
  hipEvent_t take() { return ev[next++ % 24]; }
};
std::mutex g_aux_mu;
Aux* g_aux[64][4] = {};

int aux_of(hipStream_t st, Aux** out) {
  int dev = 0;
  GNN_HIP(hipGetDevice(&dev), "hipGetDevice");
  GNN_REQUIRE(dev >= 0 && dev < 64, "gnn_train_step: device index %d", dev);
  int prio = 0, lo = 0, hi = 0;
  GNN_HIP(hipStreamGetPriority(st, &prio), "hipStreamGetPriority");
  GNN_HIP(hipDeviceGetStreamPriorityRange(&lo, &hi), "hipDeviceGetStreamPriorityRange");
  const int slot = std::min(3, std::max(0, lo - prio));
  std::lock_guard<std::mutex> g(g_aux_mu);
  Aux*& a = g_aux[dev][slot];
  if (!a) {
    std::unique_ptr<Aux> n(new Aux());
    GNN_HIP(hipStreamCreateWithPriority(&n->s, hipStreamNonBlocking, prio), "hipStreamCreateWithPriority");
    for (auto& e : n->ev) GNN_HIP(hipEventCreateWithFlags(&e, hipEventDisableTiming), "hipEventCreateWithFlags");
    a = n.release();
  }
  *out = a;
  return 0;
}

int fork_join(Aux* a, hipStream_t from, hipStream_t to) {
  hipEvent_t e = a->take();
  GNN_HIP(hipEventRecord(e, from), "hipEventRecord");
  GNN_HIP(hipStreamWaitEvent(to, e, 0), "hipStreamWaitEvent");
  return 0;
}

bool no_index() {
  const char* e = getenv("GNN_STEP_GATHER");
  const char* a = getenv("GNN_GEMM_ALGO");
  return (e && atoi(e) != 0) || (a && std::string(a) == "f32");
}

bool f32_gemm() {
  const char* e = getenv("GNN_GEMM_ALGO");
  return e && std::string(e) == "f32";
}

int pieces_of(int np) {
  if (np) return np;
  const char* e = getenv("GNN_GEMM_ALGO");
  if (!e) return 3;
  const std::string a(e);
  return a == "split2" ? 2 : a == "bf16" ? 1 : 3;
}

int gemm(int np, int ak, int bk, int64_t M, int64_t N, int64_t K, int nb, const float* const* A, int64_t lda,
         const float* const* B, int64_t ldb, float* const* C, int64_t ldc, void* ws, size_t wsb, hipStream_t st) {
  if (np == 0 && f32_gemm()) return gnn_gemm_f32(ak, bk, M, N, K, nb, A, lda, B, ldb, C, ldc, ws, wsb, st);
  return gnn_gemm_f32_split(pieces_of(np), ak, bk, M, N, K, nb, A, lda, B, ldb, C, ldc, ws, wsb, st);
}

size_t gemm_ws(int64_t M, int64_t N, int64_t K, int nb) {
  return std::max({gnn_gemm_f32_split3_workspace_bytes(M, N, K, nb), gnn_gemm_f32_workspace_bytes(M, N, K, nb),
                   gnn_gemm_f32_split_workspace_bytes(2, M, N, K, nb)});
}

bool fuse_agg_enabled() {
  const char* e = getenv("GNN_STEP_FUSE_AGG");
  return !(e && atoi(e) == 0);
}

bool small_overlap_enabled() {
  const char* e = getenv("GNN_STEP_SMALL_OVERLAP");
  return !(e && atoi(e) == 0);
}

bool overlap_enabled() {
  const char* e = getenv("GNN_STEP_OVERLAP");
  return e && atoi(e) != 0;
}

int sgemm(rocblas_handle h, rocblas_operation ta, rocblas_operation tb, int64_t m, int64_t n, int64_t k,
          const float* A, int64_t lda, const float* B, int64_t ldb, float* C, int64_t ldc) {
  const float one = 1.0f, zero = 0.0f;
  if (rocblas_sgemm(h, ta, tb, (rocblas_int)m, (rocblas_int)n, (rocblas_int)k, &one, A, (rocblas_int)lda, B,
                    (rocblas_int)ldb, &zero, C, (rocblas_int)ldc) != rocblas_status_success)
    return gnn::fail(-1, "rocblas_sgemm failed (m %lld n %lld k %lld)", (long long)m, (long long)n, (long long)k);
  return 0;
}
int mm_xwt(rocblas_handle h, const float* x, int64_t ldx, const float* W, int64_t ldw, float* out, int64_t ldo,
           int64_t M, int64_t N, int64_t K) {
  return sgemm(h, rocblas_operation_transpose, rocblas_operation_none, N, M, K, W, ldw, x, ldx, out, ldo);
}
int mm_gw(rocblas_handle h, const float* g, int64_t ldg, const float* W, int64_t ldw, float* out, int64_t ldo,
          int64_t M, int64_t K, int64_t N) {
  return sgemm(h, rocblas_operation_none, rocblas_operation_none, K, M, N, W, ldw, g, ldg, out, ldo);
}
int mm_gtx(rocblas_handle h, const float* g, int64_t ldg, const float* x, int64_t ldx, float* out, int64_t ldo,
           int64_t N, int64_t K, int64_t M) {
  return sgemm(h, rocblas_operation_none, rocblas_operation_transpose, K, N, M, x, ldx, g, ldg, out, ldo);
}

struct LayerBufs {
  int64_t M, K, nnz, F, Fk, ldx, ldo, N, D;
  bool xs_gathered;
  bool dense;
  int np;
  const float* X;
  int xk;
  const void* X16;
  float *feat, *xs, *hB, *hW, *Y, *mean, *rstd;
  float *dY, *dhB, *dhW, *dxs, *dfeat;
  void *ws_fwd, *ws_bwd, *ws_norm, *ws_gemm_f, *ws_gemm_f2, *ws_gemm_dx, *ws_gemm_dw;
  size_t b_fwd, b_bwd, b_norm, b_gemm_f, b_gemm_dx, b_gemm_dw;
  bool dy_agg;
  const int32_t *agg_rp, *agg_col, *agg_rmap;
  const float *agg_val, *agg_G, *agg_R;
  const float* in() const { return xk ? feat : X; }
  int64_t ldin() const { return xk ? ldo : ldx; }
};

struct Plan {
  int nl = 0, sage = 1;
  LayerBufs lb[GNN_STEP_MAX_LAYERS];
  float *xd, *z, *nrm, *rowloss, *lse, *dz, *dXh;
  int loss_kind = GNN_LOSS_BCE;
  uint64_t* rowmask;
  int64_t Mh = 0, Dh = 0, C = 0;
};

#define GNN_TRY(x)        \
  do {                    \
    int rc_ = (x);        \
    if (rc_) return rc_;  \
  } while (0)

int shapes(const int64_t* d, bool measuring, Plan& pl) {
  GNN_REQUIRE(d[GNN_SH_VERSION] == GNN_STEP_VERSION, "gnn_train_step: descriptor version %lld",
              (long long)d[GNN_SH_VERSION]);
  GNN_REQUIRE(d[GNN_SH_LOSS_KIND] == GNN_LOSS_BCE || d[GNN_SH_LOSS_KIND] == GNN_LOSS_CE,
              "gnn_train_step: loss kind %lld (0: BCE, 1: CE)", (long long)d[GNN_SH_LOSS_KIND]);
  pl.loss_kind = (int)d[GNN_SH_LOSS_KIND];
  pl.nl = (int)d[GNN_SH_LAYERS];
  pl.sage = d[GNN_SH_KIND] == GNN_STEP_SAGE;
  GNN_REQUIRE(pl.nl >= 1 && pl.nl <= GNN_STEP_MAX_LAYERS, "gnn_train_step: %d layers", pl.nl);
  const int64_t N = d[GNN_SH_NHID];
  const int n = pl.sage ? 2 : 1;
  for (int l = 0; l < pl.nl; ++l) {
    LayerBufs& b = pl.lb[l];
    b.dy_agg = false;
    b.M = L(d, l, GNN_SL_M);
    b.K = L(d, l, GNN_SL_K);
    b.nnz = L(d, l, GNN_SL_NNZ);
    b.N = N;
    const int64_t dense = L(d, l, GNN_SL_DENSE);
    GNN_REQUIRE(dense == 0 || dense == 1, "gnn_train_step: layer %d dense flag %lld (0: aggregating, 1: order 0)", l,
                (long long)dense);
    b.dense = dense != 0;
    const int64_t np = L(d, l, GNN_SL_GEMM);
    GNN_REQUIRE(np >= 0 && np <= 3,
                "gnn_train_step: layer %d GEMM pieces %lld (0: GNN_GEMM_ALGO, 1: bf16, 2: split2, 3: split3)", l,
                (long long)np);
    b.np = (int)np;
    b.D = b.dense ? N : n * N;
    if (b.dense) {
      GNN_REQUIRE(b.K == b.M, "gnn_train_step: order-0 layer %d has K = %lld, M = %lld", l, (long long)b.K,
                  (long long)b.M);
      b.nnz = 0;
    }
    const int64_t xk = L(d, l, GNN_SL_XKIND);
    GNN_REQUIRE(xk == GNN_FEAT_F32 || (l == 0 && (xk == GNN_FEAT_F16 || xk == GNN_FEAT_BF16)),
                "gnn_train_step: layer %d input kind %lld (0: fp32; 1 fp16 / 2 bf16 on layer 0 only)", l,
                (long long)xk);
    b.xk = (int)xk;
    b.X16 = nullptr;
    if (l == 0) {
      b.X = xk ? nullptr : HP<const float>(d, GNN_SH_X0);
      b.X16 = xk ? HP<const void>(d, GNN_SH_X0) : nullptr;
      b.ldx = d[GNN_SH_LDX0];
      b.F = d[GNN_SH_F0];
    } else {
      const LayerBufs& p = pl.lb[l - 1];
      GNN_REQUIRE(b.K == p.M, "gnn_train_step: layer %d has K = %lld, layer %d M = %lld", l, (long long)b.K, l - 1,
                  (long long)p.M);
      b.X = nullptr;
      b.ldx = p.D;
      b.F = p.D;
    }
    GNN_REQUIRE(b.F <= b.ldx && b.F > 0 && b.M > 0 && b.K > 0, "gnn_train_step: layer %d shape", l);
    b.Fk = b.F;
    if (b.F % 4 && b.ldx % 4 == 0 && (l >= 1 || (uintptr_t)b.X % 16 == 0 || measuring) &&
        b.ldx >= b.F + (4 - b.F % 4))
      b.Fk = b.F + (4 - b.F % 4);
    b.ldo = (b.Fk != b.F && b.ldx <= 2 * b.Fk) ? b.ldx : b.Fk;
    if (xk) {
      GNN_REQUIRE(b.ldx % 4 == 0 && ((uintptr_t)b.X16 % 8 == 0 || measuring),
                  "gnn_train_step: 16-bit x0 needs 8-byte aligned rows (ldx %lld)", (long long)b.ldx);
      b.Fk = (int64_t)align_up((size_t)b.F, 4);
      GNN_REQUIRE(b.Fk <= b.ldx, "gnn_train_step: 16-bit x0 rows of %lld elements have no room for %lld columns",
                  (long long)b.ldx, (long long)b.Fk);
      b.ldo = (int64_t)align_up((size_t)b.Fk, 32);
    }
    b.b_fwd = b.dense ? 0 : gnn_spmm_workspace_bytes(b.M, b.nnz, b.Fk, 0);
    b.b_gemm_f = gemm_ws(b.M, N, b.F, b.dense ? 1 : n);
  }
  const LayerBufs& top = pl.lb[pl.nl - 1];
  pl.Mh = top.M;
  pl.Dh = top.D;
  pl.C = d[GNN_SH_CLASSES];
  GNN_REQUIRE(pl.C > 0 && pl.C <= 256 && pl.Dh % 4 == 0 && pl.Dh <= 2048, "gnn_train_step: head %lld x %lld",
              (long long)pl.Dh, (long long)pl.C);
  return 0;
}

int plan_eval(const int64_t* d, Arena& ar, Plan& pl) {
  GNN_TRY(shapes(d, !ar.base, pl));
  int64_t feat = 0, xs = 0, h = 0, rows = 0, y[2] = {0, 0};
  size_t wf = 0, wg = 0;
  bool agg = false;
  for (int l = 0; l < pl.nl; ++l) {
    const LayerBufs& b = pl.lb[l];
    agg = agg || !b.dense;
    if (!b.dense || b.xk) feat = std::max(feat, b.M * b.ldo);
    if (!b.dense) xs = std::max(xs, b.M * b.ldo);
    h = std::max(h, b.M * b.N);
    rows = std::max(rows, b.M);
    y[l & 1] = std::max(y[l & 1], b.M * b.D);
    wf = std::max(wf, b.b_fwd);
    wg = std::max(wg, b.b_gemm_f);
  }
  LayerBufs s = {};
  const bool pair = pl.sage && agg;
  s.feat = (agg || feat) ? ar.take<float>(feat) : nullptr;
  s.xs = pair ? ar.take<float>(xs) : nullptr;
  s.hB = pair ? ar.take<float>(h) : nullptr;
  s.hW = ar.take<float>(h);
  float* const Y[2] = {ar.take<float>(y[0]), ar.take<float>(y[1])};
  s.mean = ar.take<float>(rows);
  s.rstd = ar.take<float>(rows);
  s.ws_fwd = agg ? ar.take<char>((int64_t)wf) : nullptr;
  s.ws_gemm_f = ar.take<char>((int64_t)wg);
  s.ws_gemm_f2 = pair ? ar.take<char>((int64_t)wg) : nullptr;
  for (int l = 0; l < pl.nl; ++l) {
    LayerBufs& b = pl.lb[l];
    if (l) b.X = pl.lb[l - 1].Y;
    b.feat = s.feat, b.xs = s.xs, b.hB = s.hB, b.hW = s.hW, b.Y = Y[l & 1], b.mean = s.mean, b.rstd = s.rstd;
    b.ws_fwd = s.ws_fwd, b.ws_gemm_f = s.ws_gemm_f, b.ws_gemm_f2 = s.ws_gemm_f2;
  }
  pl.rowloss = ar.take<float>(pl.Mh);
  pl.rowmask = ar.take<uint64_t>(pl.Mh * 8);
  return 0;
}

int plan(const int64_t* d, Arena& ar, Plan& pl) {
  GNN_TRY(shapes(d, !ar.base, pl));
  const int64_t N = d[GNN_SH_NHID];
  const int n = pl.sage ? 2 : 1;
  for (int l = 0; l < pl.nl; ++l) {
    LayerBufs& b = pl.lb[l];
    if (l) b.X = pl.lb[l - 1].Y;
    const bool pair = pl.sage && !b.dense;
    b.feat = (!b.dense || b.xk) ? ar.take<float>(b.M * b.ldo) : nullptr;
    b.xs = pair ? ar.take<float>(b.M * b.ldo) : nullptr;
    b.hB = pair ? ar.take<float>(b.M * N) : nullptr;
    b.hW = ar.take<float>(b.M * N);
    b.Y = ar.take<float>(b.M * b.D);
    b.mean = ar.take<float>(b.M);
    b.rstd = ar.take<float>(b.M);
    b.ws_fwd = b.dense ? nullptr : ar.take<char>((int64_t)b.b_fwd);
    b.ws_gemm_f = ar.take<char>((int64_t)b.b_gemm_f);
    b.ws_gemm_f2 = pair ? ar.take<char>((int64_t)b.b_gemm_f) : nullptr;
  }
  pl.xd = ar.take<float>(pl.Mh * pl.Dh);
  pl.z = ar.take<float>(pl.Mh * pl.C);
  pl.nrm = ar.take<float>(pl.Mh);
  pl.rowloss = ar.take<float>(pl.Mh);
  pl.lse = ar.take<float>(pl.Mh);
  pl.dz = ar.take<float>(pl.Mh * pl.C);
  pl.dXh = ar.take<float>(pl.Mh * pl.Dh);
  for (int l = pl.nl - 1; l >= 0; --l) {
    LayerBufs& b = pl.lb[l];
    b.dY = (l == pl.nl - 1) ? pl.dXh : nullptr;
    b.dhB = (pl.sage && !b.dense) ? ar.take<float>(b.M * N) : nullptr;
    b.dhW = ar.take<float>(b.M * N);
    b.b_norm = gnn_sage_norm_bwd_workspace_bytes(b.M, b.D);
    b.ws_norm = ar.take<char>((int64_t)b.b_norm);
    b.b_gemm_dw = gemm_ws(N, b.F, b.M, b.dense ? 1 : n);
    b.ws_gemm_dw = ar.take<char>((int64_t)b.b_gemm_dw);
    if (l >= 1 && b.dense) {
      b.dxs = b.dfeat = nullptr;
      b.b_gemm_dx = gemm_ws(b.M, b.F, N, 1);
      b.ws_gemm_dx = ar.take<char>((int64_t)b.b_gemm_dx);
      b.ws_bwd = nullptr;
      b.b_bwd = 0;
    } else if (l >= 1) {
      b.dxs = pl.sage ? ar.take<float>(b.M * b.F) : nullptr;
      b.dfeat = ar.take<float>(b.M * b.F);
      b.b_gemm_dx = gemm_ws(b.M, b.F, N, n);
      b.ws_gemm_dx = ar.take<char>((int64_t)b.b_gemm_dx);
      b.b_bwd = gnn_spmm_workspace_bytes(b.K, b.nnz, b.F, 0);
      b.ws_bwd = ar.take<char>((int64_t)b.b_bwd);
    } else {
      b.dxs = b.dfeat = nullptr;
      b.ws_gemm_dx = b.ws_bwd = nullptr;
      b.b_gemm_dx = b.b_bwd = 0;
    }
  }
  for (int l = 0; l < pl.nl - 1; ++l) pl.lb[l].dY = ar.take<float>(pl.lb[l].M * pl.lb[l].D);
  return 0;
}

struct Run {
  const int64_t* d = nullptr;
  Plan pl;
  hipStream_t st = nullptr;
  rocblas_handle h = nullptr, ha = nullptr;
  Aux* aux = nullptr;
  std::unique_lock<std::mutex> aux_lock;
  bool big_ov = false;
  float p = 0.0f;
  int training = 0;
  int64_t phase = 0;
  int64_t* T = nullptr;
  int64_t nrec = 0;

  int open(const int64_t* desc, hipStream_t stream) {
    d = desc;
    st = stream;
    GNN_TRY(blas_handle(&h));
    if (rocblas_set_stream(h, st) != rocblas_status_success) return gnn::fail(-1, "rocblas_set_stream failed");
    const int32_t bits = (int32_t)d[GNN_SH_PDROP_BITS];
    std::memcpy(&p, &bits, 4);
    big_ov = overlap_enabled() && !f32_gemm();
    const bool small_ov = small_overlap_enabled();
    if (big_ov || small_ov) GNN_TRY(aux_of(st, &aux));
    if (aux) aux_lock = std::unique_lock<std::mutex>(aux->mu);
    if (aux && small_ov) {
      GNN_TRY(blas_handle(&ha, 1));
      if (rocblas_set_stream(ha, aux->s) != rocblas_status_success) return gnn::fail(-1, "rocblas_set_stream failed");
    }
    return 0;
  }
  void arm(int64_t kind, int64_t l, int64_t M, int64_t K, int64_t nnz, int64_t F, int64_t Fk, int64_t ldx,
           int64_t ldo, const void* X, const void* Y, int64_t res_rows, int64_t xkind = 0) {
    if (!T || nrec >= T[0]) return;
    int64_t* r = T + 1 + GNN_STEP_TIMING_SLOTS * nrec++;
    gnn_spmm_set_timing_events((void*)r[0], (void*)r[1]);
    const int64_t v[] = {kind, l, M, K, nnz, F, Fk, ldx, ldo, (int64_t)(uintptr_t)X, (int64_t)(uintptr_t)Y, res_rows, 1,
                         xkind};
    std::memcpy(r + 2, v, sizeof v);
  }
  int aggregate(int l) {
    const LayerBufs& b = pl.lb[l];
    arm(0, l, b.M, b.K, b.nnz, b.F, b.Fk, b.ldx, b.ldo, b.xk ? b.X16 : (const void*)b.X, b.feat, 0, b.xk);
    const int32_t* rp = P<const int32_t>(d, l, GNN_SL_ROWPTR);
    const int32_t* col = P<const int32_t>(d, l, GNN_SL_COL);
    const float* val = P<const float>(d, l, GNN_SL_VAL);
    if (b.xk)
      return gnn_spmm_csr_h16_f32(rp, col, val, b.M, b.K, b.nnz, b.X16, b.ldx, b.xk, b.feat, b.ldo, b.Fk, b.ws_fwd,
                                  b.b_fwd, 0, st);
    return gnn_spmm_csr_f32(rp, col, val, b.M, b.K, b.nnz, b.X, b.ldx, b.feat, b.ldo, b.Fk, b.ws_fwd, b.b_fwd, 0, st);
  }
  int gather_sampled(int l, hipStream_t s) {
    const LayerBufs& b = pl.lb[l];
    const int64_t* idx = P<const int64_t>(d, l, GNN_SL_SAMPLED);
    if (b.xk) return gnn_gather_rows_h16_f32(b.X16, b.ldx, b.xk, idx, b.xs, b.ldo, nullptr, b.M, b.F, s);
    return gnn_gather_rows_f32(b.X, b.ldx, idx, b.xs, b.ldo, nullptr, b.M, b.F, s);
  }
  int stage_gate(int l) {
    if (d[GNN_SH_STAGE_EVENT] && l == (int)d[GNN_SH_STAGE_LAYER])
      GNN_HIP(hipEventRecord((hipEvent_t)d[GNN_SH_STAGE_EVENT], st), "hipEventRecord (stage gate)");
    return 0;
  }
};

int forward(Run& r) {
  const int64_t* const d = r.d;
  Plan& pl = r.pl;
  hipStream_t st = r.st;
  rocblas_handle h = r.h, ha = r.ha;
  Aux* aux = r.aux;
  const bool big_ov = r.big_ov;
  const int64_t phase = r.phase;
  const int n = pl.sage ? 2 : 1;
  for (int l = 0; l < pl.nl; ++l) {
    LayerBufs& b = pl.lb[l];
    const int64_t N = b.N;
    const float* WB = P<const float>(d, l, GNN_SL_WB);
    const float* WW = P<const float>(d, l, GNN_SL_WW);
    if (b.dense) {
      if (phase != 2 || l != 0) GNN_TRY(r.stage_gate(l));
      if (b.xk)
        GNN_TRY(gnn_gather_rows_h16_f32(b.X16, b.ldx, b.xk, nullptr, b.feat, b.ldo, nullptr, b.M, b.F, st));
      const float* X = b.in();
      const int64_t ldx = b.ldin();
      b.xs_gathered = true;
      if (gemm_ok(X, ldx) && gemm_ok(WW, b.F) && fills(b.M, N, 1)) {
        const float* A[1] = {X};
        const float* B[1] = {WW};
        float* Cc[1] = {b.hW};
        GNN_TRY(gemm(b.np, 0, 0, b.M, N, b.F, 1, A, ldx, B, b.F, Cc, N, b.ws_gemm_f, b.b_gemm_f, st));
      } else {
        GNN_TRY(mm_xwt(h, X, ldx, WW, b.F, b.hW, N, b.M, N, b.F));
      }
      GNN_TRY(gnn_sage_norm_fwd_f32(nullptr, 4, 0, b.hW, N, N, nullptr, P<const float>(d, l, GNN_SL_BW),
                                    P<const float>(d, l, GNN_SL_SCALE), P<const float>(d, l, GNN_SL_OFFSET), b.M, r.p,
                                    (uint64_t)L(d, l, GNN_SL_SEED), r.training, b.Y, b.D, b.mean, b.rstd, st));
      continue;
    }
    if (pl.sage)
      GNN_REQUIRE(L(d, l, GNN_SL_NSAMPLED) == b.M, "gnn_train_step: layer %d sampled %lld != M %lld", l,
                  (long long)L(d, l, GNN_SL_NSAMPLED), (long long)b.M);
    const bool ok = gemm_ok(b.feat, b.ldo) && gemm_ok(WW, b.F) && (!pl.sage || gemm_ok(WB, b.F));
    const bool small_side = ha && pl.sage && !(ok && fills(b.M, N, n));
    if (big_ov && pl.sage && ok && fills(b.M, N, n)) {
      b.xs_gathered = true;
      GNN_TRY(fork_join(aux, st, aux->s));
      GNN_TRY(r.gather_sampled(l, aux->s));
      const float* Ab[1] = {b.xs};
      const float* Bb[1] = {WB};
      float* Cb[1] = {b.hB};
      GNN_TRY(gnn::gemm_split3_as_batch(0, 0, b.M, N, b.F, 1, 2, 0, Ab, b.ldo, Bb, b.F, Cb, N, b.ws_gemm_f2, b.b_gemm_f,
                                        aux->s, pieces_of(b.np)));
      if (phase != 2 || l != 0) {
        GNN_TRY(r.aggregate(l));
        GNN_TRY(r.stage_gate(l));
      }
      const float* Aw[1] = {b.feat};
      const float* Bw[1] = {WW};
      float* Cw[1] = {b.hW};
      GNN_TRY(gnn::gemm_split3_as_batch(0, 0, b.M, N, b.F, 1, 2, 1, Aw, b.ldo, Bw, b.F, Cw, N, b.ws_gemm_f, b.b_gemm_f, st,
                                        pieces_of(b.np)));
      GNN_TRY(fork_join(aux, aux->s, st));
    } else if (small_side) {
      b.xs_gathered = true;
      GNN_TRY(fork_join(aux, st, aux->s));
      GNN_TRY(r.gather_sampled(l, aux->s));
      GNN_TRY(mm_xwt(ha, b.xs, b.ldo, WB, b.F, b.hB, N, b.M, N, b.F));
      if (phase != 2 || l != 0) {
        GNN_TRY(r.aggregate(l));
        GNN_TRY(r.stage_gate(l));
      }
      GNN_TRY(mm_xwt(h, b.feat, b.ldo, WW, b.F, b.hW, N, b.M, N, b.F));
      GNN_TRY(fork_join(aux, aux->s, st));
    } else {
      if (phase != 2 || l != 0) {
        GNN_TRY(r.aggregate(l));
        GNN_TRY(r.stage_gate(l));
      }
      b.xs_gathered =
          !(pl.sage && ok && fills(b.M, N, n) && b.M >= 2048 && b.ldx == b.ldo && !no_index() && !b.xk);
      if (pl.sage && b.xs_gathered) GNN_TRY(r.gather_sampled(l, st));
    }
    if ((big_ov && pl.sage && ok && fills(b.M, N, n)) || small_side) {
    } else if (ok && fills(b.M, N, n) && !b.xs_gathered) {
      const float* A[2] = {b.X, b.feat};
      const int64_t* IA[2] = {P<const int64_t>(d, l, GNN_SL_SAMPLED), nullptr};
      const float* B[2] = {WB, WW};
      float* Cc[2] = {b.hB, b.hW};
      GNN_TRY(gnn::gemm_split3_indexed(0, 0, b.M, N, b.F, n, A, b.ldo, IA, b.K, B, b.F, nullptr, 0, Cc, N,
                                       b.ws_gemm_f, b.b_gemm_f, st, pieces_of(b.np)));
    } else if (ok && fills(b.M, N, n)) {
      const float* A[2] = {pl.sage ? b.xs : b.feat, b.feat};
      const float* B[2] = {pl.sage ? WB : WW, WW};
      float* Cc[2] = {pl.sage ? b.hB : b.hW, b.hW};
      GNN_TRY(gemm(b.np, 0, 0, b.M, N, b.F, n, A + (pl.sage ? 0 : 1), b.ldo, B + (pl.sage ? 0 : 1), b.F,
                   Cc + (pl.sage ? 0 : 1), N, b.ws_gemm_f, b.b_gemm_f, st));
    } else {
      if (pl.sage) GNN_TRY(mm_xwt(h, b.xs, b.ldo, WB, b.F, b.hB, N, b.M, N, b.F));
      GNN_TRY(mm_xwt(h, b.feat, b.ldo, WW, b.F, b.hW, N, b.M, N, b.F));
    }
    GNN_TRY(gnn_sage_norm_fwd_f32(pl.sage ? b.hB : nullptr, pl.sage ? N : 4, pl.sage ? N : 0, b.hW, N, N,
                                  pl.sage ? P<const float>(d, l, GNN_SL_BB) : nullptr, P<const float>(d, l, GNN_SL_BW),
                                  P<const float>(d, l, GNN_SL_SCALE), P<const float>(d, l, GNN_SL_OFFSET), b.M, r.p,
                                  (uint64_t)L(d, l, GNN_SL_SEED), r.training, b.Y, b.D, b.mean, b.rstd, st));
  }
  return 0;
}

int check_workspace(const void* workspace, size_t workspace_bytes, size_t need) {
  GNN_REQUIRE(workspace && workspace_bytes >= need, "gnn_train_step: workspace too small (%zu < %zu)",
              workspace_bytes, need);
  GNN_REQUIRE((uintptr_t)workspace % 256 == 0, "gnn_train_step: workspace not 256-byte aligned");
  return 0;
}

}

extern "C" {

int gnn_head_bias_grad_f32(const float* dz, int64_t M, int64_t C, float* db, void* stream) {
  GNN_REQUIRE(M >= 0 && C >= 0 && M < INT_MAX && C < INT_MAX, "gnn_head_bias_grad_f32: bad size");
  if (C == 0) return 0;
  GNN_REQUIRE(db && (M == 0 || dz), "gnn_head_bias_grad_f32: NULL pointer");
  colsum_kernel<<<dim3((unsigned)C), dim3(256), 0, (hipStream_t)stream>>>(dz, (int)M, (int)C, db);
  GNN_LAUNCHED("colsum_kernel");
  return 0;
}

size_t gnn_train_step_workspace_bytes(const int64_t* desc) {
  if (!desc) return 0;
  Arena ar{nullptr};
  Plan pl;
  if (plan(desc, ar, pl)) return 0;
  return ar.off;
}

int gnn_train_step_f32(const int64_t* d, void* workspace, size_t workspace_bytes, void* stream) {
  GNN_REQUIRE(d != nullptr, "gnn_train_step: NULL descriptor");
  Arena ar{(char*)workspace};
  Run r;
  Plan& pl = r.pl;
  {
    Arena dry{nullptr};
    Plan tmp;
    GNN_TRY(plan(d, dry, tmp));
    GNN_TRY(check_workspace(workspace, workspace_bytes, dry.off));
  }
  GNN_TRY(plan(d, ar, pl));
  hipStream_t st = (hipStream_t)stream;
  GNN_TRY(r.open(d, st));
  rocblas_handle h = r.h, ha = r.ha;
  Aux* aux = r.aux;
  const bool big_ov = r.big_ov;
  const int n = pl.sage ? 2 : 1;
  const float p = r.p;
  const int training = r.training = (int)d[GNN_SH_TRAINING];
  bool aux_used = false;
  r.T = HP<int64_t>(d, GNN_SH_TIMING);
  const int64_t phase = r.phase = d[GNN_SH_PHASE];
  GNN_REQUIRE(phase >= 0 && phase <= 2, "gnn_train_step: phase %lld", (long long)phase);
  if (phase == 1) {
    r.T = nullptr;
    if (!pl.lb[0].dense) GNN_TRY(r.aggregate(0));
    return r.stage_gate(0);
  }
  GNN_TRY(forward(r));
  const LayerBufs& top = pl.lb[pl.nl - 1];
  const float* Wh = HP<const float>(d, GNN_SH_HEAD_W);
  const uint64_t hseed = (uint64_t)d[GNN_SH_HEAD_SEED];
  const float* labels = HP<const float>(d, GNN_SH_LABELS);
  const int64_t ldl = d[GNN_SH_LDL];
  const bool ce = pl.loss_kind == GNN_LOSS_CE;
  if (ce)
    GNN_TRY(gnn_head_ce_fwd_f32(top.Y, top.D, pl.Mh, pl.Dh, Wh, HP<const float>(d, GNN_SH_HEAD_B), pl.C, labels, ldl, p,
                                hseed, training, pl.xd, pl.z, pl.nrm, pl.rowloss, HP<float>(d, GNN_SH_LOSS), pl.lse,
                                st));
  else
    GNN_TRY(gnn_head_bce_fwd_f32(top.Y, top.D, pl.Mh, pl.Dh, Wh, HP<const float>(d, GNN_SH_HEAD_B), pl.C, labels, ldl,
                                 p, hseed, training, pl.xd, pl.z, pl.nrm, pl.rowloss, HP<float>(d, GNN_SH_LOSS), st));
  if (ce)
    GNN_TRY(gnn_head_ce_bwd_f32(top.Y, top.D, pl.Mh, pl.Dh, Wh, pl.C, labels, ldl, nullptr, p, hseed, training, pl.z,
                                pl.nrm, pl.dz, pl.dXh, pl.Dh, pl.lse, st));
  else
    GNN_TRY(gnn_head_bce_bwd_f32(top.Y, top.D, pl.Mh, pl.Dh, Wh, pl.C, labels, ldl, nullptr, p, hseed, training, pl.z,
                                 pl.nrm, pl.dz, pl.dXh, pl.Dh, st));
  const int64_t* const E = HP<const int64_t>(d, GNN_SH_GRAD_EVENTS);
  auto grads_ready = [&](int64_t slot, hipStream_t s) -> int {
    if (E && slot < E[0] && E[slot]) GNN_HIP(hipEventRecord((hipEvent_t)E[slot], s), "hipEventRecord (grad event)");
    return 0;
  };
  bool head_pending = true;
  auto head_grads = [&](hipStream_t s, rocblas_handle hh) -> int {
    GNN_TRY(mm_gtx(hh, pl.dz, pl.C, pl.xd, pl.Dh, HP<float>(d, GNN_SH_HEAD_GW), pl.Dh, pl.C, pl.Dh, pl.Mh));
    if (HP<float>(d, GNN_SH_HEAD_GB)) {
      colsum_kernel<<<dim3((unsigned)pl.C), dim3(256), 0, s>>>(pl.dz, (int)pl.Mh, (int)pl.C,
                                                             HP<float>(d, GNN_SH_HEAD_GB));
      GNN_LAUNCHED("colsum_kernel");
    }
    GNN_TRY(grads_ready(1, s));
    head_pending = false;
    return 0;
  };
  if (!ha) GNN_TRY(head_grads(st, h));
  for (int l = pl.nl - 1; l >= 0; --l) {
    LayerBufs& b = pl.lb[l];
    const int64_t N = b.N;
    const float* WB = P<const float>(d, l, GNN_SL_WB);
    const float* WW = P<const float>(d, l, GNN_SL_WW);
    const bool pair = pl.sage && !b.dense;
    if (b.dy_agg)
      GNN_TRY(gnn_sage_norm_bwd_agg_f32(b.agg_rp, b.agg_col, b.agg_val, b.agg_G, b.D, b.agg_R, b.D, b.agg_rmap,
                                        pair ? b.hB : nullptr, pair ? N : 4, pair ? N : 0, b.hW, N, N,
                                        pair ? P<const float>(d, l, GNN_SL_BB) : nullptr,
                                        P<const float>(d, l, GNN_SL_BW), P<const float>(d, l, GNN_SL_SCALE), b.mean,
                                        b.rstd, b.M, p, (uint64_t)L(d, l, GNN_SL_SEED), training, b.dhB, b.dhW,
                                        P<float>(d, l, GNN_SL_GSCALE), P<float>(d, l, GNN_SL_GOFFSET),
                                        pair ? P<float>(d, l, GNN_SL_GBB) : nullptr, P<float>(d, l, GNN_SL_GBW),
                                        b.ws_norm, b.b_norm, st));
    else
      GNN_TRY(gnn_sage_norm_bwd_f32(b.dY, b.D, pair ? b.hB : nullptr, pair ? N : 4, pair ? N : 0, b.hW, N, N,
                                    pair ? P<const float>(d, l, GNN_SL_BB) : nullptr, P<const float>(d, l, GNN_SL_BW),
                                    P<const float>(d, l, GNN_SL_SCALE), b.mean, b.rstd, b.M, p,
                                    (uint64_t)L(d, l, GNN_SL_SEED), training, b.dhB, b.dhW,
                                    P<float>(d, l, GNN_SL_GSCALE), P<float>(d, l, GNN_SL_GOFFSET),
                                    pair ? P<float>(d, l, GNN_SL_GBB) : nullptr, P<float>(d, l, GNN_SL_GBW),
                                    b.ws_norm, b.b_norm, st));
    if (b.dense) {
      const float* X = b.in();
      const int64_t ldx = b.ldin();
      const bool okd = gemm_ok(X, ldx) && gemm_ok(WW, b.F);
      const float* Gd[1] = {b.dhW};
      if (l >= 1) {
        float* dYp = pl.lb[l - 1].dY;
        if (okd && fills(b.M, b.F, 1)) {
          const float* B[1] = {WW};
          float* Cc[1] = {dYp};
          GNN_TRY(gemm(b.np, 0, 1, b.M, b.F, N, 1, Gd, N, B, b.F, Cc, b.F, b.ws_gemm_dx, b.b_gemm_dx, st));
        } else {
          GNN_TRY(mm_gw(h, b.dhW, N, WW, b.F, dYp, b.F, b.M, b.F, N));
        }
      }
      float* gWW = P<float>(d, l, GNN_SL_GWW);
      hipStream_t sw = st;
      if (okd && b.M >= 2048) {
        if (big_ov && l >= 1) {
          GNN_TRY(fork_join(aux, st, aux->s));
          sw = aux->s;
          aux_used = true;
        }
        const float* Xd[1] = {X};
        float* Cc[1] = {gWW};
        GNN_TRY(gemm(b.np, 1, 1, N, b.F, b.M, 1, Gd, N, Xd, ldx, Cc, b.F, b.ws_gemm_dw, b.b_gemm_dw, sw));
      } else {
        rocblas_handle hw = h;
        if (ha) {
          GNN_TRY(fork_join(aux, st, aux->s));
          sw = aux->s;
          hw = ha;
          aux_used = true;
          if (head_pending) GNN_TRY(head_grads(aux->s, ha));
        }
        GNN_TRY(mm_gtx(hw, b.dhW, N, X, ldx, gWW, b.F, N, b.F, b.M));
      }
      GNN_TRY(grads_ready(2 + l, sw));
      continue;
    }
    const bool ok = gemm_ok(b.feat, b.ldo) && gemm_ok(WW, b.F) && (!pl.sage || gemm_ok(WB, b.F));
    const float* G[2] = {pl.sage ? b.dhB : b.dhW, b.dhW};
    const int o = pl.sage ? 0 : 1;
    if (l >= 1) {
      if (ok && fills(b.M, b.F, n)) {
        const float* B[2] = {pl.sage ? WB : WW, WW};
        float* Cc[2] = {pl.sage ? b.dxs : b.dfeat, b.dfeat};
        GNN_TRY(gemm(b.np, 0, 1, b.M, b.F, N, n, G + o, N, B + o, b.F, Cc + o, b.F, b.ws_gemm_dx, b.b_gemm_dx, st));
      } else {
        if (pl.sage) GNN_TRY(mm_gw(h, b.dhB, N, WB, b.F, b.dxs, b.F, b.M, b.F, N));
        GNN_TRY(mm_gw(h, b.dhW, N, WW, b.F, b.dfeat, b.F, b.M, b.F, N));
      }
    }
    float* gWB = pl.sage ? P<float>(d, l, GNN_SL_GWB) : nullptr;
    float* gWW = P<float>(d, l, GNN_SL_GWW);
    if (ok && b.M >= 2048) {
      const float* X[2] = {pl.sage ? (b.xs_gathered ? b.xs : b.X) : b.feat, b.feat};
      const int64_t* IB[2] = {pl.sage && !b.xs_gathered ? P<const int64_t>(d, l, GNN_SL_SAMPLED) : nullptr, nullptr};
      float* Cc[2] = {pl.sage ? gWB : gWW, gWW};
      hipStream_t sw = st;
      if (big_ov && l >= 1) {
        GNN_TRY(fork_join(aux, st, aux->s));
        sw = aux->s;
        aux_used = true;
      }
      if (pl.sage && !b.xs_gathered)
        GNN_TRY(gnn::gemm_split3_indexed(1, 1, N, b.F, b.M, n, G + o, N, nullptr, 0, X + o, b.ldo, IB + o, b.K,
                                         Cc + o, b.F, b.ws_gemm_dw, b.b_gemm_dw, sw, pieces_of(b.np)));
      else
        GNN_TRY(gemm(b.np, 1, 1, N, b.F, b.M, n, G + o, N, X + o, b.ldo, Cc + o, b.F, b.ws_gemm_dw, b.b_gemm_dw, sw));
      GNN_TRY(grads_ready(2 + l, sw));
    } else {
      hipStream_t sw = st;
      rocblas_handle hw = h;
      if (ha) {
        GNN_TRY(fork_join(aux, st, aux->s));
        sw = aux->s;
        hw = ha;
        aux_used = true;
        if (head_pending) GNN_TRY(head_grads(aux->s, ha));
      }
      if (pl.sage) GNN_TRY(mm_gtx(hw, b.dhB, N, b.xs, b.ldo, gWB, b.F, N, b.F, b.M));
      GNN_TRY(mm_gtx(hw, b.dhW, N, b.feat, b.ldo, gWW, b.F, N, b.F, b.M));
      GNN_TRY(grads_ready(2 + l, sw));
    }
    if (l >= 1) {
      LayerBufs& prev = pl.lb[l - 1];
      GNN_REQUIRE(P<const int32_t>(d, l, GNN_SL_TROWPTR) != nullptr, "gnn_train_step: layer %d has no transpose", l);
      if (pl.sage) GNN_REQUIRE(P<const int32_t>(d, l, GNN_SL_RMAP) != nullptr, "gnn_train_step: layer %d has no row map", l);
      if (fuse_agg_enabled() && prev.D == b.F &&
          gnn::spmm_row_chain(b.K, b.M, b.nnz, b.F, b.F, b.F, b.dfeat, prev.dY)) {
        prev.dy_agg = true;
        prev.agg_rp = P<const int32_t>(d, l, GNN_SL_TROWPTR);
        prev.agg_col = P<const int32_t>(d, l, GNN_SL_TCOL);
        prev.agg_val = P<const float>(d, l, GNN_SL_TVAL);
        prev.agg_G = b.dfeat;
        prev.agg_R = pl.sage ? b.dxs : nullptr;
        prev.agg_rmap = pl.sage ? P<const int32_t>(d, l, GNN_SL_RMAP) : nullptr;
      } else if (pl.sage) {
        GNN_REQUIRE(P<const int32_t>(d, l, GNN_SL_RMAP) != nullptr, "gnn_train_step: layer %d has no row map", l);
        r.arm(1, l, b.K, b.M, b.nnz, b.F, b.F, b.F, b.F, b.dfeat, prev.dY, b.M);
        GNN_TRY(gnn_spmm_csr_f32_ex(P<const int32_t>(d, l, GNN_SL_TROWPTR), P<const int32_t>(d, l, GNN_SL_TCOL),
                                    P<const float>(d, l, GNN_SL_TVAL), b.K, b.M, b.nnz, b.dfeat, b.F, prev.dY, b.F,
                                    b.F, b.dxs, b.F, P<const int32_t>(d, l, GNN_SL_RMAP), b.ws_bwd, b.b_bwd, 0, st));
      } else {
        r.arm(1, l, b.K, b.M, b.nnz, b.F, b.F, b.F, b.F, b.dfeat, prev.dY, 0);
        GNN_TRY(gnn_spmm_csr_f32(P<const int32_t>(d, l, GNN_SL_TROWPTR), P<const int32_t>(d, l, GNN_SL_TCOL),
                                 P<const float>(d, l, GNN_SL_TVAL), b.K, b.M, b.nnz, b.dfeat, b.F, prev.dY, b.F, b.F,
                                 b.ws_bwd, b.b_bwd, 0, st));
      }
    }
  }
  if (head_pending) {
    GNN_TRY(fork_join(aux, st, aux->s));
    GNN_TRY(head_grads(aux->s, ha));
    aux_used = true;
  }
  if (aux_used) GNN_TRY(fork_join(aux, aux->s, st));
  return 0;
}

size_t gnn_eval_step_workspace_bytes(const int64_t* desc) {
  if (!desc) return 0;
  Arena ar{nullptr};
  Plan pl;
  if (plan_eval(desc, ar, pl)) return 0;
  return ar.off;
}

int gnn_eval_step_f32(const int64_t* d, float* logits, int64_t ldz, int32_t* counts, int mode, void* workspace,
                      size_t workspace_bytes, void* stream) {
  GNN_REQUIRE(d != nullptr, "gnn_eval_step: NULL descriptor");
  GNN_REQUIRE(d[GNN_SH_PHASE] == 0, "gnn_eval_step: phase %lld (must be 0)", (long long)d[GNN_SH_PHASE]);
  GNN_REQUIRE(mode == 0 || mode == 1, "gnn_eval_step: mode %d", mode);
  const float* labels = HP<const float>(d, GNN_SH_LABELS);
  float* loss = HP<float>(d, GNN_SH_LOSS);
  GNN_REQUIRE((labels != nullptr) == (loss != nullptr) && (!labels || counts),
              "gnn_eval_step: labels, loss and counts come together (all NULL: predict)");
  GNN_REQUIRE(labels || logits, "gnn_eval_step: nothing to produce (no labels, no logits)");
  Arena ar{(char*)workspace};
  Run r;
  Plan& pl = r.pl;
  {
    Arena dry{nullptr};
    Plan tmp;
    GNN_TRY(plan_eval(d, dry, tmp));
    GNN_TRY(check_workspace(workspace, workspace_bytes, dry.off));
    GNN_REQUIRE((!logits || ldz >= tmp.C) && (!labels || d[GNN_SH_LDL] >= tmp.C),
                "gnn_eval_step: logits / labels row stride below %lld classes", (long long)tmp.C);
  }
  GNN_TRY(plan_eval(d, ar, pl));
  GNN_TRY(r.open(d, (hipStream_t)stream));
  GNN_TRY(forward(r));
  const LayerBufs& top = pl.lb[pl.nl - 1];
  return gnn_head_eval_loss_f32(top.Y, top.D, pl.Mh, pl.Dh, HP<const float>(d, GNN_SH_HEAD_W),
                                HP<const float>(d, GNN_SH_HEAD_B), pl.C, labels, d[GNN_SH_LDL], logits, ldz,
                                pl.rowloss, pl.rowmask, loss, counts, mode, pl.loss_kind, stream);
}

}
```

### include/gnn_layers.h

```cpp
#ifndef GNN_LAYERS_H
#define GNN_LAYERS_H

#include <stddef.h>
#include <stdint.h>

#ifdef __cplusplus
extern "C" {
#endif

int gnn_sage_norm_fwd_f32(const float* hB, int64_t ldb, int64_t D1, const float* hW, int64_t ldw, int64_t D2,
                          const float* biasB, const float* biasW, const float* scale, const float* offset, int64_t M,
                          float p_drop, uint64_t seed, int training, float* Y, int64_t ldy, float* mean_out,
                          float* rstd_out, void* stream);

size_t gnn_sage_norm_bwd_workspace_bytes(int64_t M, int64_t D);

int gnn_sage_norm_bwd_f32(const float* gY, int64_t ldg, const float* hB, int64_t ldb, int64_t D1, const float* hW,
                          int64_t ldw, int64_t D2, const float* biasB, const float* biasW, const float* scale,
                          const float* mean, const float* rstd, int64_t M, float p_drop, uint64_t seed, int training,
                          float* dhB, float* dhW, float* dscale, float* doffset, float* dbiasB, float* dbiasW,
                          void* workspace, size_t workspace_bytes, void* stream);

int gnn_sage_norm_bwd_agg_f32(const int32_t* t_rowptr, const int32_t* t_col, const float* t_val, const float* G,
                              int64_t ldG, const float* R, int64_t ldr, const int32_t* rmap, const float* hB,
                              int64_t ldb, int64_t D1, const float* hW, int64_t ldw, int64_t D2, const float* biasB,
                              const float* biasW, const float* scale, const float* mean, const float* rstd, int64_t M,
                              float p_drop, uint64_t seed, int training, float* dhB, float* dhW, float* dscale,
                              float* doffset, float* dbiasB, float* dbiasW, void* workspace, size_t workspace_bytes,
                              void* stream);

int gnn_sage_norm_config(int64_t M, int64_t D, int agg, int* split_rows, int* nv, int* grid);

size_t gnn_gemm_f32_workspace_bytes(int64_t M, int64_t N, int64_t K, int nbatch);
int gnn_gemm_f32(int a_kmajor, int b_kmajor, int64_t M, int64_t N, int64_t K, int nbatch, const float* const* A,
                 int64_t lda, const float* const* B, int64_t ldb, float* const* C, int64_t ldc, void* workspace,
                 size_t workspace_bytes, void* stream);

size_t gnn_gemm_f32_split3_workspace_bytes(int64_t M, int64_t N, int64_t K, int nbatch);
int gnn_gemm_f32_split3(int a_kmajor, int b_kmajor, int64_t M, int64_t N, int64_t K, int nbatch,
                        const float* const* A, int64_t lda, const float* const* B, int64_t ldb, float* const* C,
                        int64_t ldc, void* workspace, size_t workspace_bytes, void* stream);

int gnn_gemm_f32_split3_indexed(int a_kmajor, int b_kmajor, int64_t M, int64_t N, int64_t K, int nbatch,
                                const float* const* A, int64_t lda, const int64_t* const* ia, int64_t a_rows,
                                const float* const* B, int64_t ldb, const int64_t* const* ib, int64_t b_rows,
                                float* const* C, int64_t ldc, void* workspace, size_t workspace_bytes, void* stream);

size_t gnn_gemm_f32_split_workspace_bytes(int pieces, int64_t M, int64_t N, int64_t K, int nbatch);
int gnn_gemm_f32_split(int pieces, int a_kmajor, int b_kmajor, int64_t M, int64_t N, int64_t K, int nbatch,
                       const float* const* A, int64_t lda, const float* const* B, int64_t ldb, float* const* C,
                       int64_t ldc, void* workspace, size_t workspace_bytes, void* stream);
int gnn_gemm_f32_split_indexed(int pieces, int a_kmajor, int b_kmajor, int64_t M, int64_t N, int64_t K, int nbatch,
                               const float* const* A, int64_t lda, const int64_t* const* ia, int64_t a_rows,
                               const float* const* B, int64_t ldb, const int64_t* const* ib, int64_t b_rows,
                               float* const* C, int64_t ldc, void* workspace, size_t workspace_bytes, void* stream);

size_t gnn_gemm_p3_packed_bytes(int64_t R, int64_t K);
int gnn_gemm_p3_pack_f32(const float* src, int64_t ld, int kmajor, const int64_t* idx, int64_t R, int64_t K,
                         void* out, size_t out_bytes, void* stream);
size_t gnn_gemm_p3_workspace_bytes(int64_t M, int64_t N, int64_t K, int nbatch);
int gnn_gemm_p3(int64_t M, int64_t N, int64_t K, int nbatch, const void* const* Ap, const void* const* Bp,
                float* const* C, int64_t ldc, void* workspace, size_t workspace_bytes, void* stream);

int gnn_head_bce_fwd_f32(const float* X, int64_t ldx, int64_t M, int64_t D, const float* W, const float* bias,
                         int64_t C, const float* labels, int64_t ldl, float p, uint64_t seed, int training,
                         float* xd, float* z, float* norm, float* rowloss, float* loss, void* stream);
int gnn_head_bce_bwd_f32(const float* X, int64_t ldx, int64_t M, int64_t D, const float* W, int64_t C,
                         const float* labels, int64_t ldl, const float* grad_loss, float p, uint64_t seed,
                         int training, const float* z, const float* norm, float* dz, float* dX, int64_t lddx,
                         void* stream);

int gnn_head_ce_fwd_f32(const float* X, int64_t ldx, int64_t M, int64_t D, const float* W, const float* bias,
                        int64_t C, const float* labels, int64_t ldl, float p, uint64_t seed, int training, float* xd,
                        float* z, float* norm, float* rowloss, float* loss, float* lse, void* stream);
int gnn_head_ce_bwd_f32(const float* X, int64_t ldx, int64_t M, int64_t D, const float* W, int64_t C,
                        const float* labels, int64_t ldl, const float* grad_loss, float p, uint64_t seed, int training,
                        const float* z, const float* norm, float* dz, float* dX, int64_t lddx, const float* lse,
                        void* stream);

int gnn_head_bias_grad_f32(const float* dz, int64_t M, int64_t C, float* db, void* stream);

int gnn_head_eval_f32(const float* X, int64_t ldx, int64_t M, int64_t D, const float* W, const float* bias,
                      int64_t C, const float* labels, int64_t ldl, float* z, int64_t ldz, float* rowloss,
                      uint64_t* rowmask, float* loss, int32_t* counts, int mode, void* stream);

int gnn_head_eval_loss_f32(const float* X, int64_t ldx, int64_t M, int64_t D, const float* W, const float* bias,
                           int64_t C, const float* labels, int64_t ldl, float* z, int64_t ldz, float* rowloss,
                           uint64_t* rowmask, float* loss, int32_t* counts, int mode, int loss_kind, void* stream);

#ifdef __cplusplus
}
#endif

#endif
```

### include/gnn_step.h

```cpp
#ifndef GNN_STEP_H
#define GNN_STEP_H

#include <stddef.h>
#include <stdint.h>

#ifdef __cplusplus
extern "C" {
#endif

#define GNN_STEP_VERSION 1
#define GNN_STEP_MAX_LAYERS 4
#define GNN_STEP_HEADER 24
#define GNN_STEP_LAYER_SLOTS 32
#define GNN_STEP_SAGE 0
#define GNN_STEP_GCN 1
#define GNN_STEP_TIMING_SLOTS 16
#define GNN_LOSS_BCE 0
#define GNN_LOSS_CE 1

enum {
  GNN_SH_VERSION = 0, GNN_SH_LAYERS = 1, GNN_SH_KIND = 2, GNN_SH_X0 = 3, GNN_SH_LDX0 = 4, GNN_SH_F0 = 5,
  GNN_SH_HEAD_W = 6, GNN_SH_HEAD_B = 7, GNN_SH_HEAD_GW = 8, GNN_SH_HEAD_GB = 9, GNN_SH_CLASSES = 10,
  GNN_SH_LABELS = 11, GNN_SH_LDL = 12, GNN_SH_HEAD_SEED = 13, GNN_SH_PDROP_BITS = 14, GNN_SH_TRAINING = 15,
  GNN_SH_LOSS = 16, GNN_SH_NHID = 17, GNN_SH_TIMING = 18, GNN_SH_GRAD_EVENTS = 19, GNN_SH_STAGE_EVENT = 20,
  GNN_SH_STAGE_LAYER = 21, GNN_SH_PHASE = 22, GNN_SH_LOSS_KIND = 23
};
enum {
  GNN_SL_ROWPTR = 0, GNN_SL_COL = 1, GNN_SL_VAL = 2, GNN_SL_M = 3, GNN_SL_K = 4, GNN_SL_NNZ = 5,
  GNN_SL_TROWPTR = 6, GNN_SL_TCOL = 7, GNN_SL_TVAL = 8, GNN_SL_SAMPLED = 9, GNN_SL_NSAMPLED = 10,
  GNN_SL_RMAP = 11, GNN_SL_WW = 12, GNN_SL_BW = 13, GNN_SL_WB = 14, GNN_SL_BB = 15, GNN_SL_SCALE = 16,
  GNN_SL_OFFSET = 17, GNN_SL_GWW = 18, GNN_SL_GBW = 19, GNN_SL_GWB = 20, GNN_SL_GBB = 21, GNN_SL_GSCALE = 22,
  GNN_SL_GOFFSET = 23, GNN_SL_SEED = 24, GNN_SL_XKIND = 25, GNN_SL_DENSE = 26, GNN_SL_GEMM = 27
};

size_t gnn_train_step_workspace_bytes(const int64_t* desc);
int gnn_train_step_f32(const int64_t* desc, void* workspace, size_t workspace_bytes, void* stream);

size_t gnn_eval_step_workspace_bytes(const int64_t* desc);
int gnn_eval_step_f32(const int64_t* desc, float* logits, int64_t ldz, int32_t* counts, int mode, void* workspace,
                      size_t workspace_bytes, void* stream);

#ifdef __cplusplus
}
#endif

#endif
```

Baseline: 610.2.

## Pre-pack weight matrices into split3 bf16 MFMA fragment images per step

```diff
diff --git a/gnn_amd/_lib.py b/gnn_amd/_lib.py
--- a/gnn_amd/_lib.py
+++ b/gnn_amd/_lib.py
@@ -140,6 +140,11 @@
                                   _VP]),
     "gnn_gemm_f32_split_indexed": (_INT, [_INT, _INT, _INT, _I64, _I64, _I64, _INT, _VP, _I64, _VP, _I64, _VP, _I64,
                                           _VP, _I64, _VP, _I64, _VP, _SZ, _VP]),
+    "gnn_gemm_bfrag_bytes": (_SZ, [_I64, _I64]),
+    "gnn_gemm_bfrag_pack_f32": (_INT, [_INT, _VP, _VP, _VP, _VP, _VP, _VP, _VP]),
+    "gnn_gemm_f32_split3_bfrag": (_INT, [_INT, _I64, _I64, _I64, _INT, _VP, _I64, _VP, _I64, _VP, _I64, _VP, _VP, _I64,
+                                         _VP, _SZ, _VP]),
+    "gnn_step_set_gemm_bfrag": (_INT, [_INT]),
 }
 
 EXPORTED_SYMBOLS = tuple(_SIGNATURES)
diff --git a/gnn_amd/csrc/common.h b/gnn_amd/csrc/common.h
--- a/gnn_amd/csrc/common.h
+++ b/gnn_amd/csrc/common.h
@@ -37,6 +37,13 @@
                         float* const* C, int64_t ldc, void* workspace, size_t workspace_bytes, void* stream,
                         int pieces = 3);
 
+int gemm_bfrag_pack(int count, const float* const* B, const int64_t* ldb, const int* b_kmajor, const int64_t* N,
+                    const int64_t* K, void* const* out, void* stream);
+int gemm_split3_bfrag(int b_kmajor, int64_t M, int64_t N, int64_t K, int nbatch, const float* const* A, int64_t lda,
+                      const int64_t* const* ia, int64_t a_rows, const float* const* B, int64_t ldb,
+                      const void* const* Bp, float* const* C, int64_t ldc, void* workspace, size_t workspace_bytes,
+                      void* stream);
+
 }
 
 #define GNN_REQUIRE(cond, ...)                              \
diff --git a/gnn_amd/csrc/gemm.hip b/gnn_amd/csrc/gemm.hip
--- a/gnn_amd/csrc/gemm.hip
+++ b/gnn_amd/csrc/gemm.hip
@@ -33,6 +33,7 @@
   float* C[MAX_BATCH];
   const int64_t* ia[MAX_BATCH];
   const int64_t* ib[MAX_BATCH];
+  const unsigned short* bp[MAX_BATCH];
 };
 
 template <int VEC>
@@ -409,6 +410,65 @@
   }
 }
 
+constexpr int BF_FRAG = 64 * 8;
+constexpr int BF_STEP = 3 * BF_FRAG;
+constexpr int BF_MAX_JOBS = 8;
+
+struct BfragJobs {
+  const float* src[BF_MAX_JOBS];
+  unsigned short* out[BF_MAX_JOBS];
+  int64_t ld[BF_MAX_JOBS];
+  int N[BF_MAX_JOBS], K[BF_MAX_JOBS], kmajor[BF_MAX_JOBS];
+  int first[BF_MAX_JOBS + 1];
+  int njobs;
+};
+
+__global__ __launch_bounds__(256) void bfrag_pack_kernel(BfragJobs jb) {
+  int j = 0;
+  while (j + 1 < jb.njobs && (int)blockIdx.x >= jb.first[j + 1]) ++j;
+  const int N = jb.N[j], K = jb.K[j];
+  const int KS = (K + 15) >> 4, NBLK = ((N + 127) >> 7) * 4;
+  const int u = ((int)blockIdx.x - jb.first[j]) * 256 + (int)threadIdx.x;
+  if (u >= NBLK * KS * 64) return;
+  const int lane = u & 63, fs = u >> 6;
+  const int n = (fs / KS) * 32 + (lane & 31);
+  const int kb = (fs % KS) * 16 + (lane >> 5) * 8;
+  const float* __restrict__ src = jb.src[j];
+  const int64_t ld = jb.ld[j];
+  const bool km = jb.kmajor[j] != 0;
+  float v[8];
+#pragma unroll
+  for (int i = 0; i < 8; ++i) {
+    const int k = kb + i;
+    v[i] = (n < N && k < K) ? (km ? src[(int64_t)k * ld + n] : src[(int64_t)n * ld + k]) : 0.0f;
+  }
+  u4v ph, pm, pl;
+  split8<3>(v, ph, pm, pl);
+  unsigned short* o = jb.out[j] + (int64_t)fs * BF_STEP + lane * 8;
+  *reinterpret_cast<u4v*>(o) = ph;
+  *reinterpret_cast<u4v*>(o + BF_FRAG) = pm;
+  *reinterpret_cast<u4v*>(o + 2 * BF_FRAG) = pl;
+}
+
+template <bool AK>
+__device__ __forceinline__ void s3_mma_bf(const unsigned short* __restrict__ Sa, const u4v (&fb)[2][3], int ra0, int li,
+                                          int lh, f16v (&acc)[2][2]) {
+  bf8v a[2][3];
+#pragma unroll
+  for (int p = 0; p < 3; ++p)
+#pragma unroll
+    for (int i = 0; i < 2; ++i) a[i][p] = s3_frag<AK, BM>(Sa, p, ra0 + i * 32 + li, lh);
+#pragma unroll
+  for (int q = 0; q < s3_products(3); ++q)
+#pragma unroll
+    for (int i = 0; i < 2; ++i)
+#pragma unroll
+      for (int g = 0; g < 2; ++g)
+        acc[i][g] = __builtin_amdgcn_mfma_f32_32x32x16_bf16(a[i][s3_piece_a(3, q)],
+                                                            __builtin_bit_cast(bf8v, fb[g][s3_piece_b(3, q)]),
+                                                            acc[i][g], 0, 0, 0);
+}
+
 __device__ __forceinline__ int3 xcd_tile(int gx, int gy, unsigned gz, unsigned bx, unsigned by, unsigned bz) {
   const int total = gx * gy * gz;
   const int hw = bx + gx * (by + gy * bz);
@@ -417,7 +477,7 @@
   return make_int3(lg % gx, (lg / gx) % gy, lg / (gx * gy));
 }
 
-template <bool AK, bool BKM, int VA, int VB, bool IDX, int NB, int NP = 3>
+template <bool AK, bool BKM, int VA, int VB, bool IDX, int NB, int NP = 3, bool BF = false>
 __global__ __launch_bounds__(256)
     __attribute__((amdgpu_waves_per_eu(NB == 2 ? 3 : 2, NB == 2 ? (NP == 3 ? 3 : 4) : 2))) void
 gemm_s3_kernel(Batch bt, int M, int N, int K, int64_t lda, int64_t ldb, int64_t ldc, int splits, int klen,
@@ -426,8 +486,9 @@
   constexpr int TN = 64 * NB;
   constexpr int NH = NB / 2;
   static_assert(NP >= 1 && NP <= 3 && (NP == 3 || NB == 2), "reduced piece counts: the 128 x 128 tile only");
+  static_assert(!BF || (NB == 2 && NP == 3 && !AK), "B fragments: split3's 128 x 128 tile, m-major A");
   __shared__ __attribute__((aligned(16))) unsigned short As[2][NP * S3_PIECE];
-  __shared__ __attribute__((aligned(16))) unsigned short Bs[2][NH * NP * S3_PIECE];
+  __shared__ __attribute__((aligned(16))) unsigned short Bs[2][BF ? 8 : NH * NP * S3_PIECE];
   const int t = threadIdx.x;
   const int lane = t & 63;
   const int wid = t >> 6;
@@ -466,11 +527,13 @@
   const int kend = whole ? K : min(K, kbeg + klen);
   const float* __restrict__ A = bt.A[b];
   const float* __restrict__ B = bt.B[b];
-  const __amdgpu_buffer_rsrc_t rsa = s3_rsrc(A, abytes), rsb = s3_rsrc(B, bbytes);
+  const __amdgpu_buffer_rsrc_t rsa = s3_rsrc(A, abytes),
+                               rsb = s3_rsrc(BF ? reinterpret_cast<const float*>(bt.bp[b]) : B, bbytes);
   const int64_t* __restrict__ ia = (IDX && !AK) ? bt.ia[b] : nullptr;
   const int64_t* __restrict__ ib = (IDX && BKM) ? bt.ib[b] : nullptr;
   const int voa = s3_voff<AK>(lda, m0, M, t, ia);
-  const int vob0 = s3_voff<BKM>(ldb, n0, N, t);
+  const int bf_blk = ((K + S3_BK - 1) / S3_BK) * (BF_STEP * 2);
+  const int vob0 = BF ? lane * 16 + (tx * 4 + wn * 2) * bf_blk : s3_voff<BKM>(ldb, n0, N, t);
   const int vob1 = NH == 2 ? s3_voff<BKM>(ldb, n0 + BN, N, t) : 0;
 
   const int ar = AK ? (t & 127) : (t >> 1), ah = AK ? (t >> 7) : (t & 1);
@@ -486,6 +549,7 @@
   auto load_ab = [&](int kt, float(&xa)[8], float(&xb)[8 * NH]) {
     const int k0 = kbeg + min(kt, nfull - 1) * S3_BK;
     s3_load<AK, VA, false>(rsa, A, lda, voa, m0, M, k0, kend, t, xa);
+    if constexpr (BF) return;
     if (IDX && BKM && ib)
       s3_load<BKM, VB, false, true>(rsb, B, ldb, vob0, n0, N, k0, kend, t, xb, ib);
     else
@@ -504,28 +568,46 @@
       s3_store<BKM, TN, NP>(Bs[stage], br + BN, bh, xb + 8);
     } else {
       s3_store<AK, BM, NP>(As[stage], t, xa);
-      s3_store<BKM, TN, NP>(Bs[stage], t, xb);
+      if constexpr (!BF) s3_store<BKM, TN, NP>(Bs[stage], t, xb);
     }
   };
   const int li = lane & 31, lh = lane >> 5;
+  u4v fb[2][2][3];
+  auto load_bf = [&](int step, u4v(&x)[2][3]) {
+    const int so = step * (BF_STEP * 2);
+#pragma unroll
+    for (int g = 0; g < 2; ++g)
+#pragma unroll
+      for (int p = 0; p < 3; ++p)
+        x[g][p] = __builtin_bit_cast(
+            u4v, __builtin_amdgcn_raw_buffer_load_b128(rsb, vob0 + p * (BF_FRAG * 2), so + g * bf_blk, 0));
+  };
+  auto mma = [&](int stage) {
+    if constexpr (BF) s3_mma_bf<AK>(As[stage], fb[stage], wm * 64, li, lh, acc);
+    else s3_mma<AK, BKM, NB, NP>(As[stage], Bs[stage], wm * 64, wn * (32 * NB), li, lh, acc);
+  };
+  const int sbeg = kbeg / S3_BK;
   if (nfull > 0) {
+    if constexpr (BF) load_bf(sbeg, fb[0]);
     load_ab(0, ra[0], rb[0]);
     load_ab(1, ra[1], rb[1]);
     store_ab(0, ra[0], rb[0]);
     __syncthreads();
     int kt = 0;
     for (; kt + 1 < nfull; kt += 2) {
+      if constexpr (BF) load_bf(sbeg + kt + 1, fb[1]);
       load_ab(kt + 2, ra[0], rb[0]);
-      s3_mma<AK, BKM, NB, NP>(As[0], Bs[0], wm * 64, wn * (32 * NB), li, lh, acc);
+      mma(0);
       store_ab(1, ra[1], rb[1]);
       __syncthreads();
+      if constexpr (BF) load_bf(sbeg + min(kt + 2, nfull - 1), fb[0]);
       load_ab(kt + 3, ra[1], rb[1]);
-      s3_mma<AK, BKM, NB, NP>(As[1], Bs[1], wm * 64, wn * (32 * NB), li, lh, acc);
+      mma(1);
       store_ab(0, ra[0], rb[0]);
       __syncthreads();
     }
     if (nfull & 1) {
-      s3_mma<AK, BKM, NB, NP>(As[0], Bs[0], wm * 64, wn * (32 * NB), li, lh, acc);
+      mma(0);
       __syncthreads();
     }
   }
@@ -535,7 +617,9 @@
       s3_load<AK, VA, true, true>(rsa, A, lda, voa, m0, M, k0, kend, t, ra[0], ia);
     else
       s3_load<AK, VA, true>(rsa, A, lda, voa, m0, M, k0, kend, t, ra[0]);
-    if (IDX && BKM && ib)
+    if constexpr (BF) {
+      load_bf(sbeg + nfull, fb[0]);
+    } else if (IDX && BKM && ib)
       s3_load<BKM, VB, true, true>(rsb, B, ldb, vob0, n0, N, k0, kend, t, rb[0], ib);
     else
       s3_load<BKM, VB, true>(rsb, B, ldb, vob0, n0, N, k0, kend, t, rb[0]);
@@ -547,7 +631,7 @@
     }
     store_ab(0, ra[0], rb[0]);
     __syncthreads();
-    s3_mma<AK, BKM, NB, NP>(As[0], Bs[0], wm * 64, wn * (32 * NB), li, lh, acc);
+    mma(0);
   }
 
   if constexpr (NB == 2) {
@@ -819,9 +903,15 @@
   return 0;
 }
 
+size_t bfrag_bytes(int64_t N, int64_t K) {
+  if (N <= 0 || K <= 0) return 0;
+  return (size_t)(ceil_div(N, (int64_t)128) * 4) * (size_t)ceil_div(K, (int64_t)S3_BK) * BF_STEP * 2;
+}
+
 struct Launch {
   Kern kern;
   bool idx;
+  bool bfrag;
   int np;
   int bkt;
   dim3 grid;
@@ -857,6 +947,15 @@
     else launch_s3_reduced<AK, BKM, CVA, CVB, 1>(l);
     return;
   }
+  if constexpr (!AK) {
+    if (l.bfrag) {
+      auto k = l.idx ? gemm_s3_kernel<false, false, VA, 4, true, 2, 3, true>
+                     : gemm_s3_kernel<false, false, VA, 4, false, 2, 3, true>;
+      k<<<l.grid, dim3(256), 0, l.st>>>(l.bt, l.M, l.N, l.K, l.lda, l.ldb, l.ldc, l.splits, l.klen, l.part, l.abytes,
+                                        l.bbytes, l.xcdm, l.tail_base, l.tail_s);
+      return;
+    }
+  }
   const bool wide = l.kern == KERN_S3W;
   auto k = wide ? gemm_s3_kernel<AK, BKM, VA, VB, false, 4> : gemm_s3_kernel<AK, BKM, VA, VB, false, 2>;
   if constexpr (!AK || BKM)
@@ -883,7 +982,7 @@
 int gemm_run(int algo, int a_kmajor, int b_kmajor, int64_t M, int64_t N, int64_t K, int nbatch, const float* const* A,
              int64_t lda, const float* const* B, int64_t ldb, float* const* C, int64_t ldc, void* workspace,
              size_t workspace_bytes, void* stream, int split_nbatch = 0, const RowIndex* ri = nullptr,
-             int batch_index = -1, int pieces = 3) {
+             int batch_index = -1, int pieces = 3, const void* const* Bp = nullptr) {
   GNN_REQUIRE(pieces >= 1 && pieces <= 3 && (pieces == 3 || algo == ALGO_S3),
               "gnn_gemm_f32_split: pieces %d (1: bf16, 2: split2, 3: split3)", pieces);
   GNN_REQUIRE(M >= 0 && N >= 0 && K >= 0, "gnn_gemm_f32: negative size");
@@ -907,7 +1006,11 @@
     bt.C[b] = C[b];
     bt.ia[b] = ri && ri->ia ? ri->ia[b] : nullptr;
     bt.ib[b] = ri && ri->ib ? ri->ib[b] : nullptr;
-  }
+    bt.bp[b] = Bp ? (const unsigned short*)Bp[b] : nullptr;
+    GNN_REQUIRE(!Bp || (Bp[b] && (uintptr_t)Bp[b] % 16 == 0), "gnn_gemm: B fragment image %d NULL or not 16-byte aligned", b);
+  }
+  GNN_REQUIRE(!Bp || (algo == ALGO_S3 && pieces == 3 && !a_kmajor && !(ri && ri->ib)),
+              "gnn_gemm: B fragments need split3, an m-major A and no row index on B");
   for (int b = 0; b < nbatch; ++b) l.idx = l.idx || bt.ia[b] || bt.ib[b];
   GNN_REQUIRE(!l.idx || (algo == ALGO_S3 && (!ri->ia || !a_kmajor) && (!ri->ib || b_kmajor)),
               "gnn_gemm: row indices need split3, an m-major A or a k-major B");
@@ -926,6 +1029,12 @@
   const TailPlan& tp = pl.tp;
   l.kern = pl.kern;
   l.splits = pl.splits;
+  l.bfrag = Bp && l.kern == KERN_S3 && K > 0;
+  if (l.bfrag) {
+    const size_t ib = bfrag_bytes(N, K);
+    GNN_REQUIRE(ib < (size_t)INT_MAX, "gnn_gemm: B fragment image of >= 2 GiB");
+    l.bbytes = (int64_t)ib;
+  }
   l.xcdm = xcd_map_enabled() && !(tp.s > 0 && tp.base % 8);
   l.bkt = algo == ALGO_S3 ? S3_BK : 32;
   if (algo == ALGO_F32)
@@ -1057,6 +1166,23 @@
                                   workspace, workspace_bytes, stream);
 }
 
+size_t gnn_gemm_bfrag_bytes(int64_t N, int64_t K) { return bfrag_bytes(N, K); }
+
+int gnn_gemm_bfrag_pack_f32(int count, const float* const* B, const int64_t* ldb, const int* b_kmajor,
+                            const int64_t* N, const int64_t* K, void* const* out, void* stream) {
+  return gnn::gemm_bfrag_pack(count, B, ldb, b_kmajor, N, K, out, stream);
+}
+
+int gnn_gemm_f32_split3_bfrag(int b_kmajor, int64_t M, int64_t N, int64_t K, int nbatch, const float* const* A,
+                              int64_t lda, const int64_t* const* ia, int64_t a_rows, const float* const* B,
+                              int64_t ldb, const void* const* Bp, float* const* C, int64_t ldc, void* workspace,
+                              size_t workspace_bytes, void* stream) {
+  GNN_REQUIRE(!ia || a_rows > 0, "gnn_gemm_f32_split3_bfrag: source rows");
+  GNN_REQUIRE(Bp != nullptr, "gnn_gemm_f32_split3_bfrag: NULL image array");
+  return gnn::gemm_split3_bfrag(b_kmajor, M, N, K, nbatch, A, lda, ia, a_rows, B, ldb, Bp, C, ldc, workspace,
+                                workspace_bytes, stream);
+}
+
 size_t gnn_gemm_f32_split_workspace_bytes(int pieces, int64_t M, int64_t N, int64_t K, int nbatch) {
   if (pieces < 1 || pieces > 3) return 0;
   return workspace_bytes_of(ALGO_S3, M, N, K, nbatch, pieces);
@@ -1106,4 +1232,41 @@
                   stream, 0, &ri, -1, pieces);
 }
 
-}
+int gemm_bfrag_pack(int count, const float* const* B, const int64_t* ldb, const int* b_kmajor, const int64_t* N,
+                    const int64_t* K, void* const* out, void* stream) {
+  GNN_REQUIRE(count >= 0 && (count == 0 || (B && ldb && b_kmajor && N && K && out)), "gnn_gemm_bfrag_pack_f32: arguments");
+  for (int c0 = 0; c0 < count; c0 += BF_MAX_JOBS) {
+    BfragJobs jb{};
+    int64_t wgs = 0;
+    for (int c = c0; c < count && c < c0 + BF_MAX_JOBS; ++c) {
+      if (N[c] <= 0 || K[c] <= 0) continue;
+      GNN_REQUIRE(B[c] && out[c] && (uintptr_t)out[c] % 16 == 0, "gnn_gemm_bfrag_pack_f32: matrix %d NULL or image unaligned", c);
+      GNN_REQUIRE(ldb[c] >= (b_kmajor[c] ? N[c] : K[c]), "gnn_gemm_bfrag_pack_f32: matrix %d ldb too small", c);
+      GNN_REQUIRE(bfrag_bytes(N[c], K[c]) < (size_t)INT_MAX, "gnn_gemm_bfrag_pack_f32: image of >= 2 GiB");
+      const int j = jb.njobs++;
+      jb.src[j] = B[c], jb.out[j] = (unsigned short*)out[c], jb.ld[j] = ldb[c];
+      jb.N[j] = (int)N[c], jb.K[j] = (int)K[c], jb.kmajor[j] = b_kmajor[c];
+      jb.first[j] = (int)wgs;
+      wgs += (int64_t)(bfrag_bytes(N[c], K[c]) / (BF_STEP * 2)) * 64 / 256;
+      GNN_REQUIRE(wgs < INT_MAX, "gnn_gemm_bfrag_pack_f32: too many fragments");
+    }
+    if (!jb.njobs) continue;
+    jb.first[jb.njobs] = (int)wgs;
+    bfrag_pack_kernel<<<dim3((unsigned)wgs), dim3(256), 0, (hipStream_t)stream>>>(jb);
+    GNN_LAUNCHED("bfrag_pack_kernel");
+  }
+  return 0;
+}
+
+int gemm_split3_bfrag(int b_kmajor, int64_t M, int64_t N, int64_t K, int nbatch, const float* const* A, int64_t lda,
+                      const int64_t* const* ia, int64_t a_rows, const float* const* B, int64_t ldb,
+                      const void* const* Bp, float* const* C, int64_t ldc, void* workspace, size_t workspace_bytes,
+                      void* stream) {
+  RowIndex ri;
+  ri.ia = ia;
+  ri.a_rows = a_rows;
+  return gemm_run(ALGO_S3, 0, b_kmajor, M, N, K, nbatch, A, lda, B, ldb, C, ldc, workspace, workspace_bytes, stream, 0,
+                  ia ? &ri : nullptr, -1, 3, Bp);
+}
+
+}
diff --git a/gnn_amd/csrc/step.hip b/gnn_amd/csrc/step.hip
--- a/gnn_amd/csrc/step.hip
+++ b/gnn_amd/csrc/step.hip
@@ -2,6 +2,7 @@
 #include <rocblas/rocblas.h>
 
 #include <algorithm>
+#include <atomic>
 #include <climits>
 #include <cstdint>
 #include <cstdlib>
@@ -189,6 +190,8 @@
   float *dY, *dhB, *dhW, *dxs, *dfeat;
   void *ws_fwd, *ws_bwd, *ws_norm, *ws_gemm_f, *ws_gemm_f2, *ws_gemm_dx, *ws_gemm_dw;
   size_t b_fwd, b_bwd, b_norm, b_gemm_f, b_gemm_dx, b_gemm_dw;
+  void *bf_f[2], *bf_dx[2];
+  const void *bp_f[2], *bp_dx[2];
   bool dy_agg;
   const int32_t *agg_rp, *agg_col, *agg_rmap;
   const float *agg_val, *agg_G, *agg_R;
@@ -225,6 +228,8 @@
   for (int l = 0; l < pl.nl; ++l) {
     LayerBufs& b = pl.lb[l];
     b.dy_agg = false;
+    b.bf_f[0] = b.bf_f[1] = b.bf_dx[0] = b.bf_dx[1] = nullptr;
+    b.bp_f[0] = b.bp_f[1] = b.bp_dx[0] = b.bp_dx[1] = nullptr;
     b.M = L(d, l, GNN_SL_M);
     b.K = L(d, l, GNN_SL_K);
     b.nnz = L(d, l, GNN_SL_NNZ);
@@ -383,7 +388,28 @@
     }
   }
   for (int l = 0; l < pl.nl - 1; ++l) pl.lb[l].dY = ar.take<float>(pl.lb[l].M * pl.lb[l].D);
-  return 0;
+  for (int l = 0; l < pl.nl; ++l) {
+    LayerBufs& b = pl.lb[l];
+    if (b.np != 0 && b.np != 3) continue;
+    const int nw = (pl.sage && !b.dense) ? 2 : 1;
+    for (int w = 2 - nw; w < 2; ++w) {
+      if (fills(b.M, N, nw)) b.bf_f[w] = ar.take<char>((int64_t)gnn_gemm_bfrag_bytes(N, b.F));
+      if (l >= 1 && fills(b.M, b.F, nw)) b.bf_dx[w] = ar.take<char>((int64_t)gnn_gemm_bfrag_bytes(b.F, N));
+    }
+  }
+  return 0;
+}
+
+std::atomic<int> g_bfrag{-1};
+bool bfrag_enabled() {
+  int v = g_bfrag.load(std::memory_order_relaxed);
+  if (v < 0) {
+    const char* e = getenv("GNN_GEMM_BFRAG");
+    v = !(e && atoi(e) == 0);
+    int expect = -1;
+    if (!g_bfrag.compare_exchange_strong(expect, v)) v = expect;
+  }
+  return v != 0;
 }
 
 struct Run {
@@ -449,6 +475,41 @@
     return 0;
   }
 };
+
+int pack_weights(Run& r) {
+  Plan& pl = r.pl;
+  if (!bfrag_enabled()) return 0;
+  const float* B[4 * GNN_STEP_MAX_LAYERS];
+  int64_t ld[4 * GNN_STEP_MAX_LAYERS], Nn[4 * GNN_STEP_MAX_LAYERS], Kk[4 * GNN_STEP_MAX_LAYERS];
+  int km[4 * GNN_STEP_MAX_LAYERS];
+  void* out[4 * GNN_STEP_MAX_LAYERS];
+  int c = 0;
+  for (int l = 0; l < pl.nl; ++l) {
+    LayerBufs& b = pl.lb[l];
+    if (pieces_of(b.np) != 3 || (b.np == 0 && f32_gemm())) continue;
+    const bool pair = pl.sage && !b.dense;
+    if (pair && r.big_ov) continue;
+    const float* W[2] = {pair ? P<const float>(r.d, l, GNN_SL_WB) : nullptr, P<const float>(r.d, l, GNN_SL_WW)};
+    const bool ok = b.dense ? gemm_ok(b.in(), b.ldin()) && gemm_ok(W[1], b.F)
+                            : gemm_ok(b.feat, b.ldo) && gemm_ok(W[1], b.F) && (!pair || gemm_ok(W[0], b.F));
+    if (!ok) continue;
+    const int nw = pair ? 2 : 1;
+    const bool fwd = fills(b.M, b.N, nw), dx = l >= 1 && fills(b.M, b.F, nw);
+    for (int w = 2 - nw; w < 2; ++w) {
+      if (fwd && b.bf_f[w]) {
+        B[c] = W[w], ld[c] = b.F, km[c] = 0, Nn[c] = b.N, Kk[c] = b.F, out[c] = b.bf_f[w];
+        b.bp_f[w] = b.bf_f[w];
+        ++c;
+      }
+      if (dx && b.bf_dx[w]) {
+        B[c] = W[w], ld[c] = b.F, km[c] = 1, Nn[c] = b.F, Kk[c] = b.N, out[c] = b.bf_dx[w];
+        b.bp_dx[w] = b.bf_dx[w];
+        ++c;
+      }
+    }
+  }
+  return c ? gnn::gemm_bfrag_pack(c, B, ld, km, Nn, Kk, out, r.st) : 0;
+}
 
 int forward(Run& r) {
   const int64_t* const d = r.d;
@@ -475,7 +536,11 @@
         const float* A[1] = {X};
         const float* B[1] = {WW};
         float* Cc[1] = {b.hW};
-        GNN_TRY(gemm(b.np, 0, 0, b.M, N, b.F, 1, A, ldx, B, b.F, Cc, N, b.ws_gemm_f, b.b_gemm_f, st));
+        if (b.bp_f[1])
+          GNN_TRY(gnn::gemm_split3_bfrag(0, b.M, N, b.F, 1, A, ldx, nullptr, 0, B, b.F, b.bp_f + 1, Cc, N, b.ws_gemm_f,
+                                         b.b_gemm_f, st));
+        else
+          GNN_TRY(gemm(b.np, 0, 0, b.M, N, b.F, 1, A, ldx, B, b.F, Cc, N, b.ws_gemm_f, b.b_gemm_f, st));
       } else {
         GNN_TRY(mm_xwt(h, X, ldx, WW, b.F, b.hW, N, b.M, N, b.F));
       }
@@ -534,14 +599,22 @@
       const int64_t* IA[2] = {P<const int64_t>(d, l, GNN_SL_SAMPLED), nullptr};
       const float* B[2] = {WB, WW};
       float* Cc[2] = {b.hB, b.hW};
-      GNN_TRY(gnn::gemm_split3_indexed(0, 0, b.M, N, b.F, n, A, b.ldo, IA, b.K, B, b.F, nullptr, 0, Cc, N,
-                                       b.ws_gemm_f, b.b_gemm_f, st, pieces_of(b.np)));
+      if (b.bp_f[1])
+        GNN_TRY(gnn::gemm_split3_bfrag(0, b.M, N, b.F, n, A, b.ldo, IA, b.K, B, b.F, b.bp_f, Cc, N, b.ws_gemm_f,
+                                       b.b_gemm_f, st));
+      else
+        GNN_TRY(gnn::gemm_split3_indexed(0, 0, b.M, N, b.F, n, A, b.ldo, IA, b.K, B, b.F, nullptr, 0, Cc, N,
+                                         b.ws_gemm_f, b.b_gemm_f, st, pieces_of(b.np)));
     } else if (ok && fills(b.M, N, n)) {
       const float* A[2] = {pl.sage ? b.xs : b.feat, b.feat};
       const float* B[2] = {pl.sage ? WB : WW, WW};
       float* Cc[2] = {pl.sage ? b.hB : b.hW, b.hW};
-      GNN_TRY(gemm(b.np, 0, 0, b.M, N, b.F, n, A + (pl.sage ? 0 : 1), b.ldo, B + (pl.sage ? 0 : 1), b.F,
-                   Cc + (pl.sage ? 0 : 1), N, b.ws_gemm_f, b.b_gemm_f, st));
+      const int o = pl.sage ? 0 : 1;
+      if (b.bp_f[1])
+        GNN_TRY(gnn::gemm_split3_bfrag(0, b.M, N, b.F, n, A + o, b.ldo, nullptr, 0, B + o, b.F, b.bp_f + o, Cc + o, N,
+                                       b.ws_gemm_f, b.b_gemm_f, st));
+      else
+        GNN_TRY(gemm(b.np, 0, 0, b.M, N, b.F, n, A + o, b.ldo, B + o, b.F, Cc + o, N, b.ws_gemm_f, b.b_gemm_f, st));
     } else {
       if (pl.sage) GNN_TRY(mm_xwt(h, b.xs, b.ldo, WB, b.F, b.hB, N, b.M, N, b.F));
       GNN_TRY(mm_xwt(h, b.feat, b.ldo, WW, b.F, b.hW, N, b.M, N, b.F));
@@ -572,6 +645,10 @@
   colsum_kernel<<<dim3((unsigned)C), dim3(256), 0, (hipStream_t)stream>>>(dz, (int)M, (int)C, db);
   GNN_LAUNCHED("colsum_kernel");
   return 0;
+}
+
+int gnn_step_set_gemm_bfrag(int on) {
+  return g_bfrag.exchange(on < 0 ? -1 : (on != 0), std::memory_order_relaxed);
 }
 
 size_t gnn_train_step_workspace_bytes(const int64_t* desc) {
@@ -611,6 +688,7 @@
     if (!pl.lb[0].dense) GNN_TRY(r.aggregate(0));
     return r.stage_gate(0);
   }
+  GNN_TRY(pack_weights(r));
   GNN_TRY(forward(r));
   const LayerBufs& top = pl.lb[pl.nl - 1];
   const float* Wh = HP<const float>(d, GNN_SH_HEAD_W);
@@ -682,7 +760,11 @@
         if (okd && fills(b.M, b.F, 1)) {
           const float* B[1] = {WW};
           float* Cc[1] = {dYp};
-          GNN_TRY(gemm(b.np, 0, 1, b.M, b.F, N, 1, Gd, N, B, b.F, Cc, b.F, b.ws_gemm_dx, b.b_gemm_dx, st));
+          if (b.bp_dx[1])
+            GNN_TRY(gnn::gemm_split3_bfrag(1, b.M, b.F, N, 1, Gd, N, nullptr, 0, B, b.F, b.bp_dx + 1, Cc, b.F,
+                                           b.ws_gemm_dx, b.b_gemm_dx, st));
+          else
+            GNN_TRY(gemm(b.np, 0, 1, b.M, b.F, N, 1, Gd, N, B, b.F, Cc, b.F, b.ws_gemm_dx, b.b_gemm_dx, st));
         } else {
           GNN_TRY(mm_gw(h, b.dhW, N, WW, b.F, dYp, b.F, b.M, b.F, N));
         }
@@ -719,7 +801,11 @@
       if (ok && fills(b.M, b.F, n)) {
         const float* B[2] = {pl.sage ? WB : WW, WW};
         float* Cc[2] = {pl.sage ? b.dxs : b.dfeat, b.dfeat};
-        GNN_TRY(gemm(b.np, 0, 1, b.M, b.F, N, n, G + o, N, B + o, b.F, Cc + o, b.F, b.ws_gemm_dx, b.b_gemm_dx, st));
+        if (b.bp_dx[1])
+          GNN_TRY(gnn::gemm_split3_bfrag(1, b.M, b.F, N, n, G + o, N, nullptr, 0, B + o, b.F, b.bp_dx + o, Cc + o, b.F,
+                                         b.ws_gemm_dx, b.b_gemm_dx, st));
+        else
+          GNN_TRY(gemm(b.np, 0, 1, b.M, b.F, N, n, G + o, N, B + o, b.F, Cc + o, b.F, b.ws_gemm_dx, b.b_gemm_dx, st));
       } else {
         if (pl.sage) GNN_TRY(mm_gw(h, b.dhB, N, WB, b.F, b.dxs, b.F, b.M, b.F, N));
         GNN_TRY(mm_gw(h, b.dhW, N, WW, b.F, b.dfeat, b.F, b.M, b.F, N));
diff --git a/include/gnn_layers.h b/include/gnn_layers.h
--- a/include/gnn_layers.h
+++ b/include/gnn_layers.h
@@ -62,6 +62,14 @@
 int gnn_gemm_p3(int64_t M, int64_t N, int64_t K, int nbatch, const void* const* Ap, const void* const* Bp,
                 float* const* C, int64_t ldc, void* workspace, size_t workspace_bytes, void* stream);
 
+size_t gnn_gemm_bfrag_bytes(int64_t N, int64_t K);
+int gnn_gemm_bfrag_pack_f32(int count, const float* const* B, const int64_t* ldb, const int* b_kmajor,
+                            const int64_t* N, const int64_t* K, void* const* out, void* stream);
+int gnn_gemm_f32_split3_bfrag(int b_kmajor, int64_t M, int64_t N, int64_t K, int nbatch, const float* const* A,
+                              int64_t lda, const int64_t* const* ia, int64_t a_rows, const float* const* B,
+                              int64_t ldb, const void* const* Bp, float* const* C, int64_t ldc, void* workspace,
+                              size_t workspace_bytes, void* stream);
+
 int gnn_head_bce_fwd_f32(const float* X, int64_t ldx, int64_t M, int64_t D, const float* W, const float* bias,
                          int64_t C, const float* labels, int64_t ldl, float p, uint64_t seed, int training,
                          float* xd, float* z, float* norm, float* rowloss, float* loss, void* stream);
diff --git a/include/gnn_step.h b/include/gnn_step.h
--- a/include/gnn_step.h
+++ b/include/gnn_step.h
@@ -36,6 +36,8 @@
 size_t gnn_train_step_workspace_bytes(const int64_t* desc);
 int gnn_train_step_f32(const int64_t* desc, void* workspace, size_t workspace_bytes, void* stream);
 
+int gnn_step_set_gemm_bfrag(int on);
+
 size_t gnn_eval_step_workspace_bytes(const int64_t* desc);
 int gnn_eval_step_f32(const int64_t* desc, float* logits, int64_t ldz, int32_t* counts, int mode, void* workspace,
                       size_t workspace_bytes, void* stream);
```

Measured after the change: 610.3, median of 2. No clear change (+0.0%).
